# eth-cscs/COSTA

Measured on AMD Instinct MI355X. Metric: GB/s device-resident tile pack+transpose+unpack (fp64), % HBM peak, higher is better.
Workload: dtype f64; 1 GPU; pxtran fp64 16384x16384, 256x256 blocks, op T, alpha=1 beta=0, 1x1 grid (BASELINE configs[1]); op=T, parallelism=1 rank(s), one per GPU, RCCL send/recv exchange, m=16384, n=16384, block=256, grid=1x1

## Files before the change

costa_amd/__init__.py:

```python
from __future__ import annotations

import ctypes as C
import os
import struct
from dataclasses import dataclass
from typing import Iterable, Sequence

import numpy as np

__all__ = [
    "CostaError", "lib", "FLOAT", "DOUBLE", "CFLOAT", "CDOUBLE", "INT32", "HALF", "BFLOAT16",
    "FP8_E4M3", "FP8_E5M2", "FP4_E2M1", "dtype_code", "element_code",
    "np_dtype", "Layout", "block_cyclic_layout", "custom_layout", "Comm", "transform",
    "transform_batch", "transform_async", "transform_batch_async", "synchronize", "transformer", "copy_and_transform", "execute_tiles", "execute_tiles_mixed",
    "convert_subtile", "TileOp", "TriOp", "TRI_OP_DTYPE", "transform_tri", "transform_tri_async",
    "execute_tiles_tri", "plan_export_tri", "tri_cut", "tri_subtile", "tri_phase_ms",
    "plan_export", "set_profiling", "get_stats", "release_caches", "TILE_OP_DTYPE",
    "ScaledOp", "SCALED_OP_DTYPE", "SCALED_F_ROWS", "transform_scaled", "execute_tiles_scaled",
    "plan_export_scaled", "scaled_subtile", "scaled_items",
    "transform_amax", "layout_amax", "execute_tiles_amax", "amax_items",
    "MxScales", "MX_ROWS", "MX_COLS", "MX_FLOOR", "MX_CEIL", "mx_scales", "transform_mx",
    "execute_tiles_mx", "mx_items", "mx_check_ops", "mx_check_scales",
]

# ... 85 lines not shown


class ScaledOp(C.Structure):
    _fields_ = [("op", TileOp), ("row0", C.c_int32), ("col0", C.c_int32)]


MX_ROWS, MX_COLS = 0, 1
MX_FLOOR, MX_CEIL = 0, 1


class MxScales(C.Structure):
    _fields_ = [("data", C.c_void_p), ("axis", C.c_int), ("block_stride", C.c_int64),
                ("line_stride", C.c_int64)]

    def __init__(self, data=0, axis=MX_ROWS, block_stride=0, line_stride=0):
        super().__init__(data, axis, block_stride, line_stride)


class PlanInfo(C.Structure):
    _fields_ = [("n_local", C.c_int64), ("n_pack", C.c_int64), ("n_unpack", C.c_int64),
                ("send_elems", C.c_int64), ("recv_elems", C.c_int64),
                ("local_elems", C.c_int64), ("n_ranks", C.c_int32), ("n_slots", C.c_int32)]


class TriPlanInfo(C.Structure):
    _fields_ = [("base", PlanInfo), ("n_local_tri", C.c_int64), ("n_unpack_tri", C.c_int64)]


class ScaledPlanInfo(C.Structure):
    _fields_ = [("base", PlanInfo), ("n_local_scaled", C.c_int64), ("n_unpack_scaled", C.c_int64)]


class Stats(C.Structure):
    _fields_ = [("pack_ms", C.c_double), ("local_ms", C.c_double), ("unpack_ms", C.c_double),
                ("exchange_ms", C.c_double), ("h2d_ms", C.c_double), ("d2h_ms", C.c_double),
                ("pack_launches", C.c_int64), ("local_launches", C.c_int64),
                ("unpack_launches", C.c_int64), ("pack_bytes", C.c_int64),
                ("local_bytes", C.c_int64), ("unpack_bytes", C.c_int64),
                ("transforms", C.c_int64), ("plan_hits", C.c_int64),
                ("plan_misses", C.c_int64), ("host_groups", C.c_int64),
                ("device_plans", C.c_int64), ("plan_ms", C.c_double), ("host_direct", C.c_int64),
                ("host_direct_groups", C.c_int64), ("tile_items", C.c_int64), ("skew_items", C.c_int64),
                ("cblock_items", C.c_int64), ("tiny_items", C.c_int64), ("device_lists", C.c_int64),
                ("fused_pieces", C.c_int64)]

    def as_dict(self) -> dict:
        out = {}
        for cls in reversed(type(self).__mro__):
            for k, _ in cls.__dict__.get("_fields_", ()):
                out[k] = getattr(self, k)
        return out


class FullStats(Stats):
    _fields_ = [("convert_items", C.c_int64), ("tri_items", C.c_int64)]


LIB_PATH = os.environ.get("COSTA_LIB") or os.path.join(os.path.dirname(os.path.abspath(__file__)),
                                                       "lib", "libcosta_amd.so")
_lib = None


def lib():
    global _lib
    if _lib is not None:
        return _lib
    if not os.environ.get("COSTA_NO_TORCH"):
        try:
            import torch
        except Exception:
            pass
    if not os.path.exists(LIB_PATH):
        raise CostaError(-1, f"native library missing: {LIB_PATH} (run __graft_entry__.build())")
    L = C.CDLL(LIB_PATH, mode=C.RTLD_GLOBAL)
    vp, i, c, i64 = C.c_void_p, C.c_int, C.c_char, C.c_int64
    sig = {
        "costa_hip_last_error": (C.c_char_p, []),
        "costa_hip_version": (i, []),
        "costa_hip_block_cyclic_layout": (i, [i, i, i, i, i, i, i, i, i, i, i, c, i, i, vp, i, c, i,
                                              C.POINTER(vp)]),
        "costa_hip_custom_layout": (i, [i, i, i, C.POINTER(i), C.POINTER(i), C.POINTER(i), i,
                                        C.POINTER(_Block), c, C.POINTER(vp)]),
        "costa_hip_layout_destroy": (None, [vp]),
        "costa_hip_layout_reorder_ranks": (i, [vp, C.POINTER(i), i]),
        "costa_hip_layout_num_blocks": (i, [vp]),
        "costa_hip_layout_shape": (i, [vp, C.POINTER(i), C.POINTER(i)]),
        "costa_hip_layout_block": (i, [vp, i, C.POINTER(i), C.POINTER(i), C.POINTER(i),
                                       C.POINTER(i), C.POINTER(vp), C.POINTER(i)]),
        "costa_hip_comm_self": (i, [i, C.POINTER(vp)]),
        "costa_hip_comm_unique_id": (i, [C.c_char_p]),
        "costa_hip_comm_create": (i, [C.c_char_p, i, i, i, C.POINTER(vp)]),
        "costa_hip_comm_emulated": (i, [i, i, i, C.POINTER(vp)]),
        "costa_hip_comm_emulate": (i, [vp, i, i, vp]),
        "costa_hip_exchange_rounds": (i, []),
        "costa_hip_round_range": (i, [i64, i, i, i, C.POINTER(i64), C.POINTER(i64)]),
        "costa_hip_comm_rank": (i, [vp]),
        "costa_hip_comm_size": (i, [vp]),
        "costa_hip_comm_destroy": (None, [vp]),
        "costa_hip_transform": (i, [vp, vp, c, vp, vp, vp]),
        "costa_hip_transform_batch": (i, [i, C.POINTER(vp), C.POINTER(vp), C.c_char_p, vp, vp,
                                          vp]),
        "costa_hip_transform_async": (i, [vp, vp, c, vp, vp, vp, vp]),
        "costa_hip_transform_batch_async": (i, [i, C.POINTER(vp), C.POINTER(vp), C.c_char_p, vp,
                                                vp, vp, vp]),
        "costa_hip_synchronize": (i, [vp]),
        "costa_hip_device_count": (i, [C.POINTER(i)]),
        "costa_hip_rccl_version": (i, [C.POINTER(i)]),
        "costa_hip_copy_and_transform": (i, [i, i, i, vp, i, i, vp, i, i, i, i, vp, vp]),
        "costa_hip_execute_tiles": (i, [i, C.POINTER(TileOp), i64, vp, vp, vp, i, i]),
        "costa_hip_execute_tiles_mixed": (i, [i, i, C.POINTER(TileOp), i64, vp, vp, vp, i, i]),
        "costa_hip_convert_subtile": (i, [i, i, C.POINTER(i), C.POINTER(i)]),
        "costa_hip_transform_tri": (i, [vp, vp, c, c, i, vp, vp, vp]),
        "costa_hip_transform_tri_async": (i, [vp, vp, c, c, i, vp, vp, vp, vp]),
        "costa_hip_execute_tiles_tri": (i, [i, C.POINTER(TriOp), i64, vp, vp, vp, i, i]),
        "costa_hip_tri_cut": (i, []),
        "costa_hip_tri_phase_ms": (i, [C.POINTER(C.c_double), i]),
        "costa_hip_tri_subtile": (i, [i, C.POINTER(i), C.POINTER(i)]),
        "costa_hip_plan_export_tri": (i, [vp, vp, c, c, i, vp, vp, i, i, C.POINTER(TriPlanInfo), vp, vp,
                                          vp, vp, vp, vp, vp, vp, vp, vp]),
        "costa_hip_transform_scaled": (i, [vp, vp, c, vp, vp, vp, vp, vp]),
        "costa_hip_transform_scaled_async": (i, [vp, vp, c, vp, vp, vp, vp, vp, vp]),
        "costa_hip_execute_tiles_scaled": (i, [i, i, C.POINTER(ScaledOp), i64, vp, vp, vp, i, vp, vp, i]),
        "costa_hip_scaled_subtile": (i, [i, i, C.POINTER(i), C.POINTER(i)]),
        "costa_hip_scaled_items": (i, [C.POINTER(i64), i]),
        "costa_hip_transform_amax": (i, [vp, vp, c, vp, vp, vp, vp, vp, vp, vp]),
        "costa_hip_transform_amax_async": (i, [vp, vp, c, vp, vp, vp, vp, vp, vp, vp, vp]),
        "costa_hip_layout_amax": (i, [vp, vp, vp, vp]),
        "costa_hip_layout_amax_async": (i, [vp, vp, vp, vp, vp]),
        "costa_hip_execute_tiles_amax": (i, [i, i, C.POINTER(ScaledOp), i64, vp, vp, vp, i, vp, vp, vp, vp,
                                             i]),
        "costa_hip_amax_items": (i, [C.POINTER(i64), i]),
        "costa_hip_transform_mx": (i, [vp, vp, c, vp, vp, C.POINTER(MxScales), C.POINTER(MxScales), i, vp]),
        "costa_hip_transform_mx_async": (i, [vp, vp, c, vp, vp, C.POINTER(MxScales), C.POINTER(MxScales), i,
                                             vp, vp]),
        "costa_hip_execute_tiles_mx": (i, [i, i, C.POINTER(ScaledOp), i64, vp, vp, vp, i, C.POINTER(MxScales),
                                           C.POINTER(MxScales), i, i64, i64, i, i]),
        "costa_hip_mx_items": (i, [C.POINTER(i64), i]),
        "costa_hip_mx_check_ops": (i, [C.POINTER(ScaledOp), i64, i, i64, i64]),
        "costa_hip_mx_check_scales": (i, [C.POINTER(MxScales), i64, i64]),
        "costa_hip_plan_export_scaled": (i, [vp, vp, c, vp, vp, i, i, C.POINTER(ScaledPlanInfo), vp, vp,
                                             vp, vp, vp, vp, vp, vp]),
        "costa_hip_plan_export": (i, [i, C.POINTER(vp), C.POINTER(vp), C.c_char_p, vp, vp, i, i,
                                      C.POINTER(PlanInfo), vp, vp, vp, vp, vp, vp, vp, vp]),
        "costa_hip_set_profiling": (i, [i]),
        "costa_hip_get_stats": (i, [C.POINTER(FullStats), i]),
        "costa_hip_release_caches": (i, []),
        "costa_hip_set_host_staging": (i, [i]),
        "costa_hip_set_planner": (i, [i]),
        "costa_hip_plan_export_device": (i, [i, i, C.POINTER(vp), C.POINTER(vp), C.c_char_p, vp, vp,
                                             i, i, C.POINTER(PlanInfo), vp, vp, vp, vp, vp, vp, vp,
                                             vp]),
        "costa_hip_set_list_builder": (i, [i]),
        "costa_hip_work_export": (i, [i, vp, i64, i, i, vp, i64, vp, i64, C.POINTER(i64)]),
    }
    for name, (res, args) in sig.items():
        try:
            f = getattr(L, name)
        except AttributeError:
            if os.environ.get("COSTA_LIB"):
                continue
            raise
        f.restype = res
        f.argtypes = args
    _lib = L
    return L


def _check(rc: int):
    if rc != 0:
        raise CostaError(rc, lib().costa_hip_last_error().decode(errors="replace"))


def _ptr(p) -> int:
    if p is None:
        return 0
    if isinstance(p, int):
        return p
    if isinstance(p, np.ndarray):
        return p.ctypes.data
    if hasattr(p, "data_ptr"):
        return p.data_ptr()
    raise TypeError(f"cannot take the address of {type(p)}")


def _scalar_bytes(code: int, x) -> bytes:
    if code in _FP32_SCALARS:
        code = FLOAT
    if code == DOUBLE:
        return struct.pack("<d", float(x))
    if code == CDOUBLE:
        z = complex(x)
        return struct.pack("<dd", z.real, z.imag)
    return np.asarray(x, dtype=_NP[code]).reshape(1).tobytes()


def _chr(x: str) -> C.c_char:
    return C.c_char(x.encode()[:1])


@dataclass
class BlockInfo:
    row_start: int
    row_end: int
    col_start: int
    col_end: int
    data: int
    ld: int


class Layout:

    def __init__(self, handle: int, dtype: int, keep: Iterable = ()):
        self._h = C.c_void_p(handle)
        self.dtype = dtype
        self._keep = list(keep)

    @property
    def handle(self) -> C.c_void_p:
        return self._h

    def num_blocks(self) -> int:
        return lib().costa_hip_layout_num_blocks(self._h)

    def block(self, i: int) -> BlockInfo:
        v = [C.c_int() for _ in range(4)]
        d, ld = C.c_void_p(), C.c_int()
        _check(lib().costa_hip_layout_block(self._h, i, *[C.byref(x) for x in v], C.byref(d),
                                            C.byref(ld)))
        return BlockInfo(v[0].value, v[1].value, v[2].value, v[3].value, d.value or 0, ld.value)

    def shape(self) -> tuple:
        m, n = C.c_int(), C.c_int()
        _check(lib().costa_hip_layout_shape(self._h, C.byref(m), C.byref(n)))
        return m.value, n.value

    def reorder_ranks(self, reordering: Sequence[int]):
        p = np.ascontiguousarray(reordering, dtype=np.int32)
        _check(lib().costa_hip_layout_reorder_ranks(self._h, p.ctypes.data_as(C.POINTER(C.c_int)),
                                                    int(p.size)))

    def close(self):
        if self._h and self._h.value:
            lib().costa_hip_layout_destroy(self._h)
            self._h = C.c_void_p(0)

    def __del__(self):
        try:
            self.close()
        except Exception:
            pass


def block_cyclic_layout(m, n, block_m, block_n, i, j, sub_m, sub_n, p_m, p_n, order, rsrc, csrc,
                        ptr, lld, ordering, rank, dtype=DOUBLE) -> Layout:
    code = element_code(dtype)
    h = C.c_void_p()
    _check(lib().costa_hip_block_cyclic_layout(code, m, n, block_m, block_n, i, j, sub_m, sub_n,
                                               p_m, p_n, _chr(order), rsrc, csrc,
                                               C.c_void_p(_ptr(ptr)), lld, _chr(ordering), rank,
                                               C.byref(h)))
    return Layout(h.value, code, [ptr])


def custom_layout(rowblocks, colblocks, rowsplit, colsplit, owners, localblocks, ordering,
                  dtype=DOUBLE) -> Layout:
    code = element_code(dtype)
    rs = np.ascontiguousarray(rowsplit, dtype=np.int32)
    cs = np.ascontiguousarray(colsplit, dtype=np.int32)
    ow = np.ascontiguousarray(owners, dtype=np.int32).reshape(-1)
    lb = list(localblocks)
    arr = np.zeros(max(1, len(lb)), _BLOCK_DTYPE)
    if lb:
        arr["data"][:len(lb)] = [_ptr(b[0]) for b in lb]
        rest = np.asarray([b[1:4] for b in lb], dtype=np.int64).reshape(len(lb), 3)
        arr["ld"][:len(lb)] = rest[:, 0]
        arr["row"][:len(lb)] = rest[:, 1]
        arr["col"][:len(lb)] = rest[:, 2]
    h = C.c_void_p()
    ip = C.POINTER(C.c_int)
    _check(lib().costa_hip_custom_layout(code, rowblocks, colblocks, rs.ctypes.data_as(ip),
                                         cs.ctypes.data_as(ip), ow.ctypes.data_as(ip), len(lb),
                                         arr.ctypes.data_as(C.POINTER(_Block)), _chr(ordering),
                                         C.byref(h)))
    return Layout(h.value, code, [b[0] for b in lb])


EMULATE_PACK, EMULATE_UNPACK, EMULATE_LOCAL = 1, 2, 3
EMULATE_PARTS = {"pack": EMULATE_PACK, "unpack": EMULATE_UNPACK, "local": EMULATE_LOCAL}


def exchange_rounds() -> int:
    return lib().costa_hip_exchange_rounds()


def round_range(count: int, elem_bytes: int, rounds: int, round: int) -> tuple:
    lo, hi = C.c_int64(), C.c_int64()
    _check(lib().costa_hip_round_range(count, elem_bytes, rounds, round, C.byref(lo), C.byref(hi)))
    return lo.value, hi.value


class Comm:

    def __init__(self, handle: int):
        self._h = C.c_void_p(handle)

    @staticmethod
# ... 434 lines not shown
        rows, cols = shape
        along, lines = (rows, cols) if ax == MX_ROWS else (cols, rows)
        want = ((along + 31) // 32, lines)
        if tuple(tensor.shape) != want:
            raise ValueError(f"mx_scales: shape {tuple(tensor.shape)}, the matrix needs {want} "
                             "([blocks, lines])")
    bs, ls = tensor.stride()
    if (tensor.shape[0] > 1 and bs <= 0) or (tensor.shape[1] > 1 and ls <= 0):
        raise ValueError("mx_scales: the strides must be positive")
    d = MxScales(tensor.data_ptr(), ax, max(bs, 1), max(ls, 1))
    d._keep = tensor
    return d


def _mx_arg(d, what, shape=None):
    if d is None:
        return None
    if not isinstance(d, MxScales):
        raise ValueError(f"{what}: an MxScales descriptor (costa.mx_scales(tensor, axis)), not {type(d)}")
    t = getattr(d, "_keep", None)
    if t is not None and shape is not None:
        rows, cols = shape
        along, lines = (rows, cols) if d.axis == MX_ROWS else (cols, rows)
        want = ((along + 31) // 32, lines)
        if tuple(t.shape) != want:
            raise ValueError(f"{what}: shape {tuple(t.shape)}, the {rows} x {cols} matrix needs {want} "
                             "([blocks, lines])")
    return C.byref(d)


def transform_mx(A: Layout, Cl: Layout, comm: Comm, trans: str = "N", alpha=1.0, beta=0.0,
                 a_scales=None, c_scales=None, rounding="floor", stream=None):
    if not isinstance(A, Layout) or not isinstance(Cl, Layout):
        raise CostaError(1, "costa: batches of MX layout pairs are not supported")
    code = _scalar_code(A.dtype, Cl.dtype)
    ab, bb = _scalar_bytes(code, alpha), _scalar_bytes(code, beta)
    args = (A.handle, Cl.handle, _chr(trans), ab, bb, _mx_arg(a_scales, "a_scales", A.shape()),
            _mx_arg(c_scales, "c_scales", Cl.shape()), _mx_rounding(rounding), comm.handle)
    if stream is None:
        _check(lib().costa_hip_transform_mx(*args))
    else:
        s = getattr(stream, "cuda_stream", stream) or 0
        _check(lib().costa_hip_transform_mx_async(*args, C.c_void_p(s)))


def execute_tiles_mx(src_dtype, dst_dtype, ops: np.ndarray, scalars: np.ndarray, m: int, n: int,
                     src_base=0, dst_base=0, a_scales=None, c_scales=None, rounding="floor",
                     a_transposed: bool = False, device: int = 0):
    sc_, dc_ = element_code(src_dtype), element_code(dst_dtype)
    ops = np.ascontiguousarray(ops, dtype=SCALED_OP_DTYPE)
    sc = np.ascontiguousarray(scalars, dtype=np.float32).reshape(-1)
    assert sc.size % 2 == 0
    _check(lib().costa_hip_execute_tiles_mx(sc_, dc_, ops.ctypes.data_as(C.POINTER(ScaledOp)), ops.size,
                                            C.c_void_p(_ptr(src_base)), C.c_void_p(_ptr(dst_base)),
                                            sc.ctypes.data, sc.size // 2, _mx_arg(a_scales, "a_scales"),
                                            _mx_arg(c_scales, "c_scales"), _mx_rounding(rounding), m, n,
                                            int(a_transposed), device))


def mx_items(reset: bool = False) -> int:
    v = C.c_int64(0)
    _check(lib().costa_hip_mx_items(C.byref(v), int(reset)))
    return v.value


def mx_check_ops(ops: np.ndarray, axis, m: int, n: int):
    ops = np.ascontiguousarray(ops, dtype=SCALED_OP_DTYPE)
    _check(lib().costa_hip_mx_check_ops(ops.ctypes.data_as(C.POINTER(ScaledOp)), ops.size, _mx_axis(axis),
                                        m, n))


def mx_check_scales(d: MxScales, rows: int, cols: int):
    _check(lib().costa_hip_mx_check_scales(C.byref(d), rows, cols))


@dataclass
class ScaledPlan(Plan):
    local_scaled: np.ndarray = None
    unpack_scaled: np.ndarray = None


def plan_export_scaled(A: Layout, Cl: Layout, rank: int, nranks: int, trans: str = "N", alpha=1,
                       beta=0) -> ScaledPlan:
    if not isinstance(A, Layout) or not isinstance(Cl, Layout):
        raise CostaError(1, "costa: batches of scaled layout pairs are not supported")
    code = _scalar_code(A.dtype, Cl.dtype)
    ab, bb = _scalar_bytes(code, alpha), _scalar_bytes(code, beta)
    info = ScaledPlanInfo()
    L = lib()
    args = (A.handle, Cl.handle, _chr(trans), ab, bb, rank, nranks, C.byref(info))
    _check(L.costa_hip_plan_export_scaled(*args, *([None] * 8)))
    b = info.base
    po = np.zeros(b.n_pack, TILE_OP_DTYPE)
    ls = np.zeros(info.n_local_scaled, SCALED_OP_DTYPE)
    us = np.zeros(info.n_unpack_scaled, SCALED_OP_DTYPE)
    cnt = [np.zeros(nranks, np.int64) for _ in range(4)]
    sc = np.zeros(2 * b.n_slots, _NP[code])
    _check(L.costa_hip_plan_export_scaled(*args, po.ctypes.data, ls.ctypes.data, us.ctypes.data,
                                          *[x.ctypes.data for x in cnt], sc.ctypes.data))
    return ScaledPlan(np.zeros(b.n_local, TILE_OP_DTYPE), po, np.zeros(b.n_unpack, TILE_OP_DTYPE), *cnt,
                      sc, b.send_elems, b.recv_elems, b.local_elems, ls, us)


def set_profiling(on: bool = True):
    _check(lib().costa_hip_set_profiling(int(on)))


def get_stats(reset: bool = False) -> dict:
    s = FullStats()
    _check(lib().costa_hip_get_stats(C.byref(s), int(reset)))
    return s.as_dict()


def release_caches():
    _check(lib().costa_hip_release_caches())


def set_planner(mode: int):
    _check(lib().costa_hip_set_planner(int(mode)))


def set_list_builder(mode: int):
    _check(lib().costa_hip_set_list_builder(int(mode)))


@dataclass
class WorkLists:
    ordered: np.ndarray
    work: np.ndarray
    meta: dict
    on_gpu: bool


_WORK_META = ("n_large", "n_medium", "n_skew", "n_cblock", "cblock_lds", "cb_map", "tiny_first",
              "n_tiny", "n_ordered", "n_work", "on_gpu", "flags")


def work_export(dtype, ops: np.ndarray, kind: str = "local", device=None) -> WorkLists:
    code = element_code(dtype)
    ops = np.ascontiguousarray(ops, dtype=TILE_OP_DTYPE)
    k = {"local": 0, "pack": 1, "unpack": 2}[kind]
    dev = -1 if device is None else int(device)
    meta = (C.c_int64 * 12)()
    L = lib()
    _check(L.costa_hip_work_export(code, ops.ctypes.data, ops.size, k, dev, None, 0, None, 0, meta))
    o = np.zeros(meta[8], TILE_OP_DTYPE)
    w = np.zeros(meta[9], np.uint64)
    _check(L.costa_hip_work_export(code, ops.ctypes.data, ops.size, k, dev, o.ctypes.data, o.size,
                                   w.ctypes.data, w.size, meta))
    m = dict(zip(_WORK_META, list(meta)))
    return WorkLists(o, w, m, bool(m["on_gpu"]))


def set_host_staging(mode: int):
    _check(lib().costa_hip_set_host_staging(int(mode)))


def rccl_version() -> int:
    v = C.c_int(0)
    _check(lib().costa_hip_rccl_version(C.byref(v)))
    return v.value
```

costa_amd/csrc/capi.cpp:

```cpp
#include "engine.hpp"

#include <hip/hip_runtime.h>

#include <costa/transform.hpp>

#include <algorithm>
#include <cctype>
#include <complex>
#include <cstring>
#include <new>

struct costa_layout_s {
    costa::engine::elayout e;
    std::vector<int> base_owners;
};
struct costa_comm_s {
    costa::engine::comm* c = nullptr;
};

namespace {
thread_local std::string g_last_error;

template <typename F>
int guarded(F&& f) {
// ... 695 lines not shown
            throw costa::engine::error(COSTA_ERR_ARG, "bad rank/size");
        check_handles(1, &A, &C);
        auto jobs = make_scaled_job(A, C, trans, alpha, beta, nullptr, nullptr);
        if (costa::engine::dtype_is_fp4(A->e.dtype) || costa::engine::dtype_is_fp4(C->e.dtype)) jobs[0].mx = true;
        auto p = costa::engine::make_plan(jobs, rank, nranks);
        info->base.n_local = int64_t(p->local_ops.size());
        info->base.n_pack = int64_t(p->pack_ops.size());
        info->base.n_unpack = int64_t(p->unpack_ops.size());
        info->base.send_elems = p->send_elems;
        info->base.recv_elems = p->recv_elems;
        info->base.local_elems = p->local_elems;
        info->base.n_ranks = nranks;
        info->base.n_slots = int32_t(p->slots.size());
        info->n_local_scaled = int64_t(p->local_scaled.size());
        info->n_unpack_scaled = int64_t(p->unpack_scaled.size());
        auto cp = [](const auto& v, auto* dst) {
            if (dst && !v.empty()) std::memcpy(dst, v.data(), v.size() * sizeof(v[0]));
        };
        cp(p->pack_ops, pack_ops);
        cp(p->local_scaled, local_scaled);
        cp(p->unpack_scaled, unpack_scaled);
        cp(p->send_counts, send_counts);
        cp(p->send_displs, send_displs);
        cp(p->recv_counts, recv_counts);
        cp(p->recv_displs, recv_displs);
        if (scalars) {
            const size_t E = dtype_size(p->scalar_dtype());
            auto* out = static_cast<unsigned char*>(scalars);
            std::memcpy(out, p->slots[0].alpha.data(), E);
            std::memcpy(out + E, p->slots[0].beta.data(), E);
        }
    });
}

int costa_hip_synchronize(costa_comm_t comm) {
    return gpu_guarded([&] {
        if (!comm) throw costa::engine::error(COSTA_ERR_ARG, "null communicator");
        costa::engine::synchronize(comm->c);
    });
}

int costa_hip_copy_and_transform(costa_dtype_t dtype, int n_rows, int n_cols, const void* src,
                                 int src_stride, int src_col_major, void* dst, int dst_stride,
                                 int dst_col_major, int transpose, int conjugate,
                                 const void* alpha, const void* beta) {
    return gpu_guarded([&] {
        if (!alpha || !beta) throw costa::engine::error(COSTA_ERR_ARG, "null scalar");
        costa::engine::copy_and_transform(dtype, n_rows, n_cols, src, src_stride, src_col_major != 0,
                                          dst, dst_stride, dst_col_major != 0, transpose != 0,
                                          conjugate != 0, alpha, beta);
    });
}

int costa_hip_execute_tiles(costa_dtype_t dtype, const costa_tile_op_t* ops, int64_t n,
                            const void* src_base, void* dst_base, const void* scalars,
                            int n_slots, int device) {
    return gpu_guarded([&] {
        if (n < 0 || (n > 0 && (!ops || !scalars)))
            throw costa::engine::error(COSTA_ERR_ARG, "null argument");
        costa::engine::execute_tiles(dtype, ops, n, src_base, dst_base, scalars, n_slots, device);
    });
}

int costa_hip_execute_tiles_mixed(costa_dtype_t src_dtype, costa_dtype_t dst_dtype,
                                  const costa_tile_op_t* ops, int64_t n, const void* src_base,
                                  void* dst_base, const void* scalars, int n_slots, int device) {
    return gpu_guarded([&] {
        if (n < 0 || (n > 0 && (!ops || !scalars)))
            throw costa::engine::error(COSTA_ERR_ARG, "null argument");
        costa::engine::execute_tiles_mixed(src_dtype, dst_dtype, ops, n, src_base, dst_base, scalars,
                                           n_slots, device);
    });
}

int costa_hip_convert_subtile(costa_dtype_t src_dtype, costa_dtype_t dst_dtype, int* bf, int* bs) {
    return guarded([&] {
        if (!bf || !bs) throw costa::engine::error(COSTA_ERR_ARG, "null argument");
        costa::engine::convert_subtile(src_dtype, dst_dtype, bf, bs);
    });
}

int costa_hip_plan_export(int n, const costa_layout_t* A, const costa_layout_t* C,
                          const char* trans, const void* alpha, const void* beta, int rank,
                          int nranks, costa_plan_info_t* info, costa_tile_op_t* local_ops,
                          costa_tile_op_t* pack_ops, costa_tile_op_t* unpack_ops,
                          int64_t* send_counts, int64_t* send_displs, int64_t* recv_counts,
                          int64_t* recv_displs, void* scalars) {
    return export_plan(
        [&](const std::vector<job>& jobs) { return costa::engine::make_plan(jobs, rank, nranks); },
        n, A, C, trans, alpha, beta, rank, nranks, info, local_ops, pack_ops, unpack_ops,
        send_counts, send_displs, recv_counts, recv_displs, scalars);
}

int costa_hip_plan_export_device(int device, int n, const costa_layout_t* A, const costa_layout_t* C,
                                 const char* trans, const void* alpha, const void* beta, int rank,
                                 int nranks, costa_plan_info_t* info, costa_tile_op_t* local_ops,
                                 costa_tile_op_t* pack_ops, costa_tile_op_t* unpack_ops,
                                 int64_t* send_counts, int64_t* send_displs, int64_t* recv_counts,
                                 int64_t* recv_displs, void* scalars) {
    device_restore keep;
    return export_plan(
        [&](const std::vector<job>& jobs) {
            auto p = costa::engine::make_plan_device(jobs, rank, nranks, 0, device, nullptr);
            if (!p)
                throw costa::engine::error(COSTA_ERR_ARG,
                                           "costa: the device planner does not apply to these "
                                           "layouts (local blocks are not exactly the rank's grid "
                                           "cells)");
            return p;
        },
        n, A, C, trans, alpha, beta, rank, nranks, info, local_ops, pack_ops, unpack_ops,
        send_counts, send_displs, recv_counts, recv_displs, scalars);
}

int costa_hip_set_planner(int mode) {
    return guarded([&] {
        if (mode < 0 || mode > 2) throw costa::engine::error(COSTA_ERR_ARG, "mode must be 0, 1 or 2");
        costa::engine::set_planner_mode(mode);
    });
}

int costa_hip_set_list_builder(int mode) {
    return guarded([&] {
        if (mode < 0 || mode > 2) throw costa::engine::error(COSTA_ERR_ARG, "mode must be 0, 1 or 2");
        costa::engine::set_list_builder_mode(mode);
    });
}

int costa_hip_work_export(int dtype, const costa_tile_op_t* ops, int64_t n_ops, int kind, int device,
                          costa_tile_op_t* ordered, int64_t cap_ordered, uint64_t* work,
                          int64_t cap_work, int64_t* meta) {
    auto body = [&] {
        if (!meta || (n_ops > 0 && !ops) || n_ops < 0) throw costa::engine::error(COSTA_ERR_ARG, "null argument");
        if (dtype < COSTA_FLOAT || dtype > COSTA_INT32) throw costa::engine::error(COSTA_ERR_ARG, "bad dtype");
        if (kind < 0 || kind > 2) throw costa::engine::error(COSTA_ERR_ARG, "kind must be 0, 1 or 2");
        std::vector<costa_tile_op_t> in(ops, ops + n_ops), o;
        std::vector<uint64_t> w;
        costa::engine::work_split ws;
        const bool on_gpu = costa::engine::work_export(
            costa_dtype_t(dtype), in, costa::engine::list_kind(kind), device, o, w, ws);
        const int64_t m[12] = {ws.n_large, ws.n_medium, ws.n_skew, ws.n_cblock, ws.cblock_lds, ws.cb_map,
                               ws.tiny_first, ws.n_tiny, int64_t(o.size()), int64_t(w.size()), on_gpu,
                               int64_t(ws.tr_shape) | int64_t(ws.sq) << 1 | int64_t(ws.full) << 2 |
                                   int64_t(ws.med_full) << 3 | int64_t(ws.med_sq) << 4 |
                                   int64_t(ws.skew_wide) << 5};
        std::memcpy(meta, m, sizeof(m));
        if (ordered && cap_ordered >= int64_t(o.size()) && !o.empty())
            std::memcpy(ordered, o.data(), o.size() * sizeof(o[0]));
        if (work && cap_work >= int64_t(w.size()) && !w.empty()) std::memcpy(work, w.data(), w.size() * sizeof(w[0]));
    };
    return device >= 0 ? gpu_guarded(body) : guarded(body);
}

int costa_hip_set_profiling(int on) {
    costa::engine::set_profiling(on != 0);
    return COSTA_OK;
}

int costa_hip_get_stats(costa_stats_t* out, int reset) {
    return guarded([&] {
        if (!out) throw costa::engine::error(COSTA_ERR_ARG, "null argument");
        costa::engine::resolve_pending();
        *out = costa::engine::stats();
        if (reset) costa::engine::stats() = costa_stats_t{};
    });
}

int costa_hip_set_host_staging(int mode) {
    return guarded([&] {
        if (mode != 0 && mode != 1) throw costa::engine::error(COSTA_ERR_ARG, "mode must be 0 or 1");
        costa::engine::set_host_staging_mode(mode);
    });
}

int costa_hip_release_caches(void) {
    return gpu_guarded([&] { costa::engine::release_caches(); });
}

}

namespace costa {
namespace {
void raise(int rc) {
    if (rc != COSTA_OK) throw hip_error(rc, g_last_error);
}
template <typename T>
engine::scal scal_of(T a, T b) {
    engine::scal s;
    std::memcpy(s.alpha.data(), &a, sizeof(T));
    std::memcpy(s.beta.data(), &b, sizeof(T));
    return s;
}
template <typename T>
void run(std::vector<layout_ref<T>>& from, std::vector<layout_ref<T>>& to, const char* trans,
         const T* alpha, const T* beta, costa_comm_t comm) {
    raise(gpu_guarded([&] {
        if (from.size() != to.size())
            throw engine::error(COSTA_ERR_ARG, "costa::transform: from/to sizes differ");
        if (!comm) throw engine::error(COSTA_ERR_ARG, "costa::transform: null communicator");
        std::vector<engine::elayout> es;
        es.reserve(2 * from.size());
        std::vector<engine::job> jobs(from.size());
        for (size_t i = 0; i < from.size(); ++i) {
            es.push_back(engine::erase(from[i].get()));
            jobs[i].A = &es.back();
            es.push_back(engine::erase(to[i].get()));
            jobs[i].C = &es.back();
            jobs[i].trans = trans ? trans[i] : 'N';
            jobs[i].s = alpha ? scal_of(alpha[i], beta[i]) : scal_of(T{1}, T{0});
        }
        engine::transform(jobs, comm->c);
    }));
}
}

template <typename T>
void transform(grid_layout<T>& A, grid_layout<T>& C, costa_comm_t comm) {
    std::vector<layout_ref<T>> f{A}, t{C};
    run<T>(f, t, nullptr, nullptr, nullptr, comm);
}

template <typename T>
void transform(grid_layout<T>& A, grid_layout<T>& C, char trans, T alpha, T beta,
               costa_comm_t comm) {
    std::vector<layout_ref<T>> f{A}, t{C};
    run<T>(f, t, &trans, &alpha, &beta, comm);
}

template <typename T>
void transform(std::vector<layout_ref<T>>& from, std::vector<layout_ref<T>>& to,
               costa_comm_t comm) {
    run<T>(from, to, nullptr, nullptr, nullptr, comm);
}

template <typename T>
void transform(std::vector<layout_ref<T>>& from, std::vector<layout_ref<T>>& to, const char* trans,
               const T* alpha, const T* beta, costa_comm_t comm) {
    run<T>(from, to, trans, alpha, beta, comm);
}

template <typename T>
void transform_triangular(grid_layout<T>& A, grid_layout<T>& C, char trans, char uplo, int k, T alpha,
                          T beta, costa_comm_t comm) {
    raise(gpu_guarded([&] {
        if (!comm) throw engine::error(COSTA_ERR_ARG, "costa::transform_triangular: null communicator");
        const char ul = char(std::toupper(static_cast<unsigned char>(uplo)));
        if (ul != 'U' && ul != 'L')
            throw engine::error(COSTA_ERR_ARG, "costa::transform_triangular: uplo must be 'U' or 'L'");
        engine::elayout a = engine::erase(A), c = engine::erase(C);
        engine::job jb;
        jb.A = &a;
        jb.C = &c;
        jb.trans = trans;
        jb.s = scal_of(alpha, beta);
        jb.uplo = ul;
        jb.k = k;
        engine::transform({jb}, comm->c);
    }));
}
#define COSTA_INSTANTIATE_TRI(T)                                                                  \
    template void transform_triangular<T>(grid_layout<T>&, grid_layout<T>&, char, char, int, T, T, \
                                          costa_comm_t);
COSTA_INSTANTIATE_TRI(float)
COSTA_INSTANTIATE_TRI(double)
COSTA_INSTANTIATE_TRI(std::complex<float>)
COSTA_INSTANTIATE_TRI(std::complex<double>)
COSTA_INSTANTIATE_TRI(int)

template <typename Ta, typename Tc>
void run_mixed(grid_layout<Ta>& A, grid_layout<Tc>& C, char trans, Tc alpha, Tc beta,
               costa_comm_t comm) {
    raise(gpu_guarded([&] {
        if (!comm) throw engine::error(COSTA_ERR_ARG, "costa::transform: null communicator");
        engine::elayout a = engine::erase(A), c = engine::erase(C);
        engine::job jb;
        jb.A = &a;
        jb.C = &c;
        jb.trans = trans;
        jb.s = scal_of(alpha, beta);
        engine::transform({jb}, comm->c);
    }));
}

template <typename Ta, typename Tc>
typename std::enable_if<!std::is_same<Ta, Tc>::value>::type
transform(grid_layout<Ta>& A, grid_layout<Tc>& C, costa_comm_t comm) {
    run_mixed<Ta, Tc>(A, C, 'N', Tc{1}, Tc{0}, comm);
}

template <typename Ta, typename Tc>
typename std::enable_if<!std::is_same<Ta, Tc>::value>::type
transform(grid_layout<Ta>& A, grid_layout<Tc>& C, char trans, Tc alpha, Tc beta, costa_comm_t comm) {
    run_mixed<Ta, Tc>(A, C, trans, alpha, beta, comm);
}

#define COSTA_INSTANTIATE_MIXED(Ta, Tc)                                                         \
    template void transform<Ta, Tc>(grid_layout<Ta>&, grid_layout<Tc>&, costa_comm_t);          \
    template void transform<Ta, Tc>(grid_layout<Ta>&, grid_layout<Tc>&, char, Tc, Tc, costa_comm_t);

COSTA_INSTANTIATE_MIXED(double, float)
COSTA_INSTANTIATE_MIXED(float, double)
COSTA_INSTANTIATE_MIXED(std::complex<double>, std::complex<float>)
COSTA_INSTANTIATE_MIXED(std::complex<float>, std::complex<double>)

#define COSTA_INSTANTIATE_TRANSFORM(T)                                                          \
    template void transform<T>(grid_layout<T>&, grid_layout<T>&, costa_comm_t);                 \
// ... 14 lines not shown
```

costa_amd/csrc/device_lists.hip:

```cpp
#include <hip/hip_runtime.h>
#include <rocprim/device/device_radix_sort.hpp>
#include <rocprim/device/device_scan.hpp>
#include <rocprim/device/device_scan_by_key.hpp>

#include <algorithm>
#include <chrono>
#include <cstdio>
#include <cstdlib>

#include "engine.hpp"

namespace costa {
namespace engine {

#define DL_CHECK(x)                                                                    \
    do {                                                                               \
        hipError_t e_ = (x);                                                           \
        if (e_ != hipSuccess)                                                          \
            throw error(COSTA_ERR_HIP, std::string(#x " failed: ") + hipGetErrorString(e_)); \
    } while (0)

namespace {

using u64 = unsigned long long;
// ... 530 lines not shown
    DL_CHECK(hipMemcpyAsync(d_ops, ops_h.data(), ops_h.size() * sizeof(costa_tile_op_t), hipMemcpyHostToDevice, s));
    DL_CHECK(hipMemcpyAsync(d_wave, wave_h.data(), N * 4, hipMemcpyHostToDevice, s));
    DL_CHECK(hipMemcpyAsync(d_t, &th, sizeof(th), hipMemcpyHostToDevice, s));
    DL_CHECK(hipMemsetAsync(odd, 0, N * 4, s));
    DL_CHECK(hipMemsetAsync(bad, 0, N * 4, s));
    DL_CHECK(hipMemsetAsync(taken, 0, N, s));
    hipLaunchKernelGGL(dl_candidates, dim3(dl_grid(nw)), dim3(kThreads), 0, s, d_ops, d_wave, nw, E, budget, flag,
                       lo, hi, ldd, d_t);
    DL_CHECK(hipGetLastError());
    scan_u32(flag, pos, N);
    hipLaunchKernelGGL(dl_compact, dim3(dl_grid(nw)), dim3(kThreads), 0, s, flag, pos, nw, cand, d_t);
    DL_CHECK(hipGetLastError());
    DL_CHECK(hipMemcpyAsync(&th, d_t, sizeof(th), hipMemcpyDeviceToHost, s));
    sync();
    lap[0] = now() - t0;
    const int64_t nc = int64_t(th.ncand);
    if (nc < 2) return 0;
    const uint64_t lo_min = th.lo_min;
    const int sb = bits_of((th.lo_max - lo_min) / uint64_t(E)), lb = bits_of(uint64_t(budget));
    const int hb = bits_of((th.hi_max - lo_min) / uint64_t(E));
    if (sb + lb > 64 || hb + lb > 64) return -1;
    const size_t NC = size_t(nc);

    hipLaunchKernelGGL(dl_keys, dim3(dl_grid(nc)), dim3(kThreads), 0, s, cand, nc, lo, ldd, lo_min, E, sb, key, va);
    DL_CHECK(hipGetLastError());
    sort_u64(key, NC, sb + lb, sval, ka, kb, va, vb);
    hipLaunchKernelGGL(dl_gather, dim3(dl_grid(nc)), dim3(kThreads), 0, s, sval, cand, d_wave, nc, lo, hi, ldd, s_i,
                       s_op, s_lo, s_hi, s_ldd);
    hipLaunchKernelGGL(dl_rhi, dim3(dl_grid(nc)), dim3(kThreads), 0, s, s_ldd, s_hi, nc, lo_min, E, hb, rhi);
    DL_CHECK(hipGetLastError());
    max_u64(rhi, pmax, NC);
    hipLaunchKernelGGL(dl_starts, dim3(dl_grid(nc)), dim3(kThreads), 0, s, s_lo, s_ldd, pmax, nc, lo_min, E, hb,
                       start);
    DL_CHECK(hipGetLastError());
    scan_u32(start, cnum, NC);
    hipLaunchKernelGGL(dl_inclusive, dim3(dl_grid(nc)), dim3(kThreads), 0, s, start, nc, cnum);
    hipLaunchKernelGGL(dl_bounds, dim3(dl_grid(nc)), dim3(kThreads), 0, s, start, cnum, nc, comp_a, comp_b, d_t);
    hipLaunchKernelGGL(dl_check, dim3(dl_grid(nc)), dim3(kThreads), 0, s, d_ops, s_op, s_lo, s_ldd, comp_a, comp_b, nc,
                       E, vec_bits, comp_K, comp_fl, comp_ok, d_t);
    DL_CHECK(hipGetLastError());
    DL_CHECK(hipMemcpyAsync(&th, d_t, sizeof(th), hipMemcpyDeviceToHost, s));
    sync();
    lap[1] = now() - t0;
    const uint64_t ncomp = th.ncomp;
    if (th.ck_max == 0) return 0;
    const int ck = bits_of(th.ck_max), cb = bits_of(ncomp);
    if (ck + cb > 64) return -1;

    hipLaunchKernelGGL(dl_corners, dim3(dl_grid(nc)), dim3(kThreads), 0, s, d_ops, s_op, s_lo, s_ldd, cnum, comp_a,
                       comp_ok, comp_K, nc, E, ck, ncomp, ckeys);
    DL_CHECK(hipGetLastError());
    sort_u64(ckeys, 4 * NC, ck + cb, perm, ka, kb, va, vb);
    hipLaunchKernelGGL(dl_gather_u64, dim3(dl_grid(4 * nc)), dim3(kThreads), 0, s, ckeys, perm, 4 * nc, sckeys);
    hipLaunchKernelGGL(dl_parity, dim3(dl_grid(4 * nc)), dim3(kThreads), 0, s, sckeys, 4 * nc, ck, ncomp, s_ldd,
                       comp_a, comp_K, odd, bad);
    hipLaunchKernelGGL(dl_count, dim3(dl_grid(nc)), dim3(kThreads), 0, s, comp_ok, odd, bad, s_ldd, comp_a, comp_K,
                       budget, nc, comp_ng, comp_KB, d_t);
    DL_CHECK(hipGetLastError());
    scan_i64(comp_ng, comp_gat, NC);
    hipLaunchKernelGGL(dl_total, dim3(1), dim3(64), 0, s, comp_ng, comp_gat, d_t);
    DL_CHECK(hipGetLastError());
    DL_CHECK(hipMemcpyAsync(&th, d_t, sizeof(th), hipMemcpyDeviceToHost, s));
    sync();
    lap[2] = now() - t0;
    const int64_t ng = int64_t(th.ng);
    if (ng == 0) return 0;
    if (ng > int64_t(UINT32_MAX)) return -1;
    const size_t G = size_t(ng);

    dl_mem mg;
    const size_t o_gc = mg.take(G * 8), o_gc2 = mg.take(G * 8), o_gd = mg.take(G * 8), o_gb = mg.take(G * 4);
    const size_t o_gn = mg.take(G * 4), o_gh = mg.take(G * 4), o_gk = mg.take(G * 8);
    const size_t o_io = mg.take(G * 4), o_o1 = mg.take(G * 4), o_by = mg.take(G * 4), o_sh = mg.take(G * 4);
    const size_t o_bd = mg.take(G * 4), o_bk = mg.take(G * 4), o_sbk = mg.take(G * 4), o_ord = mg.take(G * 4);
    const size_t o_sz = mg.take(G * 8), o_at = mg.take(G * 8);
    const size_t o_gka = mg.take(G * 4), o_gkb = mg.take(G * 4), o_gva = mg.take(G * 4), o_gvb = mg.take(G * 4);
    mg.alloc();
    uint64_t *g_comp0 = mg.at<uint64_t>(o_gc), *g_comp = mg.at<uint64_t>(o_gc2), *g_dst = mg.at<uint64_t>(o_gd);
    uint32_t *g_band = mg.at<uint32_t>(o_gb), *g_nops = mg.at<uint32_t>(o_gn), *g_hint = mg.at<uint32_t>(o_gh);
    uint64_t* gkey = mg.at<uint64_t>(o_gk);
    uint32_t *iota = mg.at<uint32_t>(o_io), *order1 = mg.at<uint32_t>(o_o1), *by = mg.at<uint32_t>(o_by);
    uint32_t *shint = mg.at<uint32_t>(o_sh), *slice = mg.at<uint32_t>(o_bd), *bkey = mg.at<uint32_t>(o_bk);
    uint32_t *sbkey = mg.at<uint32_t>(o_sbk), *order = mg.at<uint32_t>(o_ord);
    uint64_t *gsize = mg.at<uint64_t>(o_sz), *gat = mg.at<uint64_t>(o_at);
    uint32_t *gka = mg.at<uint32_t>(o_gka), *gkb = mg.at<uint32_t>(o_gkb), *gva = mg.at<uint32_t>(o_gva);
    uint32_t* gvb = mg.at<uint32_t>(o_gvb);

    DL_CHECK(hipMemsetAsync(g_comp0, 0, G * 8, s));
    hipLaunchKernelGGL(dl_seed, dim3(dl_grid(nc)), dim3(kThreads), 0, s, comp_ng, comp_gat, nc, g_comp0, d_t);
    DL_CHECK(hipGetLastError());
    max_u64(g_comp0, g_comp, G);
    hipLaunchKernelGGL(dl_table, dim3(dl_grid(ng)), dim3(kThreads), 0, s, d_ops, s_op, s_lo, s_ldd, comp_a, comp_b,
                       comp_K, comp_KB, comp_fl, comp_gat, g_comp, ng, E, g_dst, g_band, g_nops, g_hint, d_t);
    hipLaunchKernelGGL(dl_taken, dim3(dl_grid(nc)), dim3(kThreads), 0, s, cnum, comp_ng, s_i, nc, taken);
    hipLaunchKernelGGL(dl_dst_keys, dim3(dl_grid(ng)), dim3(kThreads), 0, s, g_dst, ng, lo_min, E, gkey, iota);
    DL_CHECK(hipGetLastError());
    sort_u64(gkey, G, hb, order1, gka, gkb, gva, gvb);
    DL_CHECK(hipMemcpyAsync(&th, d_t, sizeof(th), hipMemcpyDeviceToHost, s));
    sync();
    lap[3] = now() - t0;
    const bool any_tr = th.any_tr != 0, hints = th.hints_bad == 0;
    lds = int64_t(th.lds);
    map = any_tr ? cb_xcd_chunks : cb_round_robin;
    const bool bands = bands_env == 1 || (bands_env == -1 && !any_tr);
    const uint32_t* final_order = order1;
    if (bands && ng >= 16 && hints) {
        hipLaunchKernelGGL(dl_iota, dim3(dl_grid(ng)), dim3(kThreads), 0, s, ng, iota);
        DL_CHECK(hipGetLastError());
        sort_u32(g_hint, shint, iota, by, G, 32);
        hipLaunchKernelGGL(dl_slices, dim3(dl_grid(ng)), dim3(kThreads), 0, s, by, ng, slice);
        hipLaunchKernelGGL(dl_gather_u32, dim3(dl_grid(ng)), dim3(kThreads), 0, s, slice, order1, ng, bkey);
        DL_CHECK(hipGetLastError());
        sort_u32(bkey, sbkey, order1, order, G, 3);
        final_order = order;
        map = cb_xcd_bands;
    }

    hipLaunchKernelGGL(dl_sizes, dim3(dl_grid(ng)), dim3(kThreads), 0, s, final_order, g_nops, ng, gsize);
    DL_CHECK(hipGetLastError());
    scan_i64(gsize, gat, G);
    hipLaunchKernelGGL(dl_out_total, dim3(1), dim3(64), 0, s, gat, gsize, ng, d_t);
    DL_CHECK(hipGetLastError());
    DL_CHECK(hipMemcpyAsync(&th, d_t, sizeof(th), hipMemcpyDeviceToHost, s));
    sync();
    lap[4] = now() - t0;
    const size_t n_out = size_t(th.n_out);
    void* out = nullptr;
    const size_t out_ops_bytes = (n_out * sizeof(costa_tile_op_t) + 255) & ~size_t(255);
    DL_CHECK(hipMalloc(&out, out_ops_bytes + G * 8));
    sec.mem = std::shared_ptr<void>(out, [](void* p) { (void)hipFree(p); });
    sec.d_ordered = static_cast<costa_tile_op_t*>(out);
    sec.d_work = reinterpret_cast<uint64_t*>(static_cast<char*>(out) + out_ops_bytes);
    hipLaunchKernelGGL(dl_emit, dim3(dl_grid(ng)), dim3(kThreads), 0, s, d_ops, s_op, s_lo, s_ldd, comp_a, comp_b,
                       comp_K, comp_KB, comp_fl, g_comp, g_band, g_nops, g_dst, final_order, gat, ng, E,
                       uint64_t(base_at), sec.d_ordered, sec.d_work);
    DL_CHECK(hipGetLastError());
    DL_CHECK(hipMemcpyAsync(taken_h.data(), taken, N, hipMemcpyDeviceToHost, s));
    sync();
    sec.at_ordered = base_at;
    sec.n_ordered = n_out;
    sec.n_work = G;
    if (trace) {
        lap[5] = now() - t0;
        std::fprintf(stderr,
                     "[costa device groups] %lld candidates, %llu components (%llu / %llu checked, %llu stray, %llu four), %lld groups: upload + candidates "
                     "%.2f ms, order + components + check %.2f, corners + counts %.2f, group table + order "
                     "%.2f, slices + sizes %.2f, emit %.2f\n",
                     (long long)nc, (unsigned long long)ncomp, th.n_ok, th.n_valid, th.n_bad, th.n_odd4, (long long)ng, lap[0], lap[1] - lap[0],
                     lap[2] - lap[1], lap[3] - lap[2], lap[4] - lap[3], lap[5] - lap[4]);
    }
    return ng;
}

}
}
```

costa_amd/csrc/engine.cpp:

```cpp
#include <exception>
#include <thread>
#include "engine.hpp"
#include "strip_work.hpp"

#include <hip/hip_runtime.h>
#include <rccl/rccl.h>

#include <algorithm>
#include <numeric>
#include <chrono>
#include <cmath>
#include <cstdio>
#include <cstdlib>
#include <cstring>
#include <deque>
#include <list>
#include <map>
#include <mutex>
#include <unordered_map>

namespace costa {
namespace engine {

#define HIP_CHECK(x)                                                                   \
// ... 1239 lines not shown
                key[x] = {((op.dst + uint64_t((fp * op.ldd + s0) * E)) << 6) | uint64_t((f0 - fp) / bf), wx};
            }
            std::sort(key.begin(), key.end());
            const size_t n = key.size(), blk = size_t(8 * F);
            for (size_t b = 0; b < n; b += blk) {
                const size_t m = std::min(blk, n - b);
                for (size_t x = 0; x < m; ++x) {
                    const size_t run = x / size_t(F), in = x % size_t(F);
                    const size_t to = m == blk ? in * 8 + run : x;
                    work[w0 + b + to] = key[b + x].second;
                }
            }
        }
        n_work[c] = int64_t(work.size() - w0);
    }
    lap(0);
    int64_t cblock_lds = 0;
    int cb_map = cb_round_robin;
    const int64_t n_cblock = cblock_groups(dtype, wave_ops, kind, ordered, work, cblock_lds, cb_map, ops, dev);
    const size_t n_dev = dev ? dev->n_ordered : 0;
    lap(1);
    const size_t nw = wave_ops.size();
    uint32_t top = 0;
    bool tr = false;
    for (const auto* o : wave_ops) {
        top = std::max(top, o->order);
        tr = tr || (o->flags & COSTA_TILE_TRANSPOSE);
    }
    const int mode = kn.sort == 5   ? (pack_list ? 1 : 2)
                     : kn.sort == 4 ? (tr || top == 0 ? 2 : 3)
                     : kn.sort == 3 && top == 0 ? 2 : kn.sort;
    std::vector<uint32_t> perm(nw);
    if (mode == 3 && size_t(top) <= 4 * nw + 1024) {
        std::vector<uint32_t> at(size_t(top) + 2, 0);
        for (const auto* o : wave_ops) ++at[size_t(o->order) + 1];
        for (size_t k = 1; k < at.size(); ++k) at[k] += at[k - 1];
        for (size_t i = 0; i < nw; ++i) perm[at[wave_ops[i]->order]++] = uint32_t(i);
    } else if (mode == 2 && nw > 0) {
        uint64_t lo = ~uint64_t(0), hi = 0;
        for (const auto* o : wave_ops) {
            lo = std::min(lo, o->dst);
            hi = std::max(hi, o->dst);
        }
        std::vector<uint64_t> key(nw), key2(nw);
        std::vector<uint32_t> idx2(nw);
        for (size_t i = 0; i < nw; ++i) {
            key[i] = (wave_ops[i]->dst - lo) / uint64_t(E);
            perm[i] = uint32_t(i);
        }
        const uint64_t span = (hi - lo) / uint64_t(E);
        constexpr int B = 14;
        std::vector<uint32_t> at((1 << B) + 1);
        for (int shift = 0; shift == 0 || (shift < 64 && (span >> shift) != 0); shift += B) {
            std::fill(at.begin(), at.end(), 0u);
            for (size_t i = 0; i < nw; ++i) ++at[((key[i] >> shift) & ((1 << B) - 1)) + 1];
            for (int d = 1; d <= (1 << B); ++d) at[d] += at[d - 1];
            for (size_t i = 0; i < nw; ++i) {
                const uint32_t p = at[(key[i] >> shift) & ((1 << B) - 1)]++;
                key2[p] = key[i];
                idx2[p] = perm[i];
            }
            key.swap(key2);
            perm.swap(idx2);
        }
    } else if (mode >= 1 && mode <= 3) {
        std::vector<std::pair<uint64_t, uint32_t>> key(nw);
        for (size_t i = 0; i < nw; ++i) {
            const costa_tile_op_t& o = *wave_ops[i];
            key[i] = {mode == 1 ? o.src : mode == 2 ? o.dst : o.order, uint32_t(i)};
        }
        std::sort(key.begin(), key.end());
        for (size_t i = 0; i < nw; ++i) perm[i] = key[i].second;
    } else {
        for (size_t i = 0; i < nw; ++i) perm[i] = uint32_t(i);
    }
    if (kn.xcd_bands && mode == 2 && top > 0 && nw > 1) xcd_bands(wave_ops, E, kn.xcd_bands, local, perm);
    lap(2);
    std::vector<wave_grid> grid(nw);
    std::vector<size_t> at_piece(nw + 1, 0);
    host_parallel(nw, [&](size_t b, size_t e) {
        for (size_t i = b; i < e; ++i) grid[i] = wave_pieces(*wave_ops[perm[i]], E, local);
    });
    for (size_t i = 0; i < nw; ++i)
        at_piece[i + 1] = at_piece[i] + size_t(grid[i].nfc * grid[i].nsc);
    work_split w;
    w.tr_shape = tr_shape;
    w.sq = sq;
    w.full = tr_shape && !sq && !shaped[0].empty();
    for (const uint32_t li : shaped[0]) {
        const costa_tile_op_t& op = ops[li];
        w.full = w.full && (op.flags & vec_both) == vec_both && op.nf % sh.bf == 0 && op.ns % sh.bs == 0;
    }
    w.med_sq = med_sq && !shaped[1].empty();
    w.med_full = !shaped[1].empty() && n_work[1] > 0 && !w.med_sq;
    for (const uint32_t li : shaped[1])
        w.med_full = w.med_full && ops[li].nf % sh.bf_m == 0 && ops[li].ns % sh.bs_m == 0;
    w.n_large = n_work[0];
    w.n_medium = n_work[1];
    w.n_skew = n_work[2];
    w.skew_wide = skew_wide && n_work[2] > 0;
    w.n_cblock = n_cblock;
    w.cblock_lds = cblock_lds;
    w.cb_map = cb_map;

    w.tiny_first = int64_t(ordered.size() + n_dev);
    w.n_tiny = int64_t(at_piece[nw]);
    const size_t base = ordered.size();
    ordered.resize(base + at_piece[nw]);
    host_parallel(nw, [&](size_t b, size_t e) {
        for (size_t i = b; i < e; ++i)
            emit_pieces(*wave_ops[perm[i]], E, grid[i], local, &ordered[base + at_piece[i]]);
    });
    if (trace) {
        lap(3);
        std::fprintf(stderr,
                     "[costa build_work] %zu ops (%s list): classify + shaped %.2f ms (merge %.2f, flags + "
                     "granules %.2f, classify %.2f, work items %.2f), groups %.2f (%lld), "
                     "wavefront order %.2f, pieces %.2f (%lld)\n",
                     ops_in.size(), pack_list ? "pack" : local ? "local" : "unpack", bw_t[0], sub_t[0],
                     sub_t[1] - sub_t[0], sub_t[2] - sub_t[1], bw_t[0] - sub_t[2], bw_t[1] - bw_t[0],
                     (long long)n_cblock, bw_t[2] - bw_t[1], bw_t[3] - bw_t[2], (long long)w.n_tiny);
    }
    return w;
}

launch_args make_launch(const work_split& w, const void* d_ordered, const void* d_work,
                        const char* src_base, char* dst_base, const void* d_scalars, bool transpose,
                        bool axpby) {
    launch_args a;
    a.ops = static_cast<const costa_tile_op_t*>(d_ordered);
    a.work = static_cast<const uint64_t*>(d_work);
    a.n_large = w.n_large;
    a.n_medium = w.n_medium;
    a.n_skew = w.n_skew;
    a.n_cblock = w.n_cblock;
    a.cblock_lds = w.cblock_lds;
    a.cb_map = w.cb_map;
    a.tiny_first = w.tiny_first;
    a.n_tiny = w.n_tiny;
    a.src_base = src_base;
    a.dst_base = dst_base;
    a.scalars = d_scalars;
    a.any_transpose = transpose;
    a.any_axpby = axpby;
    a.tr_shape = w.tr_shape;
    a.sq = w.sq;
    a.full = w.full;
    a.med_full = w.med_full;
    a.med_sq = w.med_sq;
    a.skew_wide = w.skew_wide;
    return a;
}

namespace {

struct hrange {
    uintptr_t lo, hi;
    size_t dev_off;
};

size_t block_extent_bytes(const eblock& b, char ordering, size_t E) {
    const int64_t nr = b.rows.length(), nc = b.cols.length();
    if (nr == 0 || nc == 0) return 0;
    const int64_t fast = ordering == 'R' ? nc : nr, slow = ordering == 'R' ? nr : nc;
    return size_t((slow - 1) * int64_t(b.ld) + fast) * E;
}

bool is_device_ptr(const void* p) {
    hipPointerAttribute_t a;
    hipError_t e = hipPointerGetAttributes(&a, p);
    if (e != hipSuccess) {
        (void)hipGetLastError();
        return false;
    }
    return a.type == hipMemoryTypeDevice;
}

bool layout_on_device(const elayout& L) {
    if (L.blocks.empty()) return true;
    bool first = is_device_ptr(L.blocks.front().data);
    uintptr_t lo = 0, hi = 0;
    for (const auto& b : L.blocks) {
        uintptr_t p = reinterpret_cast<uintptr_t>(b.data);
        if (first && p >= lo && p < hi) continue;
        bool d = is_device_ptr(b.data);
        if (d != first)
            throw error(COSTA_ERR_ARG, "costa: a layout mixes host and device blocks");
        if (d) {
            hipDeviceptr_t base = nullptr;
            size_t sz = 0;
            if (hipMemGetAddressRange(&base, &sz, const_cast<char*>(b.data)) == hipSuccess) {
                lo = reinterpret_cast<uintptr_t>(base);
                hi = lo + sz;
            } else {
                (void)hipGetLastError();
            }
        }
    }
    return first;
}

}

namespace {
int g_host_mode = -1;
}
int host_staging_mode() {
    if (g_host_mode < 0) {
        const char* s = std::getenv("COSTA_HOST_STAGING");
        g_host_mode = s ? (std::atoi(s) != 0) : 1;
    }
    return g_host_mode;
}
void set_host_staging_mode(int mode) {
    std::lock_guard<std::recursive_mutex> lk(g_mutex);
    g_host_mode = mode != 0;
}

namespace {

struct hasher {
    uint64_t h = 0x9E3779B97F4A7C15ull;
    uint64_t h2 = 0x2545F4914F6CDD1Dull;
    void mix(uint64_t v) {
        v ^= v >> 33;
        v *= 0xff51afd7ed558ccdull;
        v ^= v >> 33;
        h = (h ^ v) * 0xc4ceb9fe1a85ec53ull + 0x165667b19e3779f9ull;
        h ^= h >> 29;
        h2 = (h2 + v) * 0x9fb21c651e98df25ull;
        h2 ^= h2 >> 31;
    }
    void mix_vec(const std::vector<int>& v) {
        mix(v.size());
        for (int x : v) mix(uint64_t(uint32_t(x)));
    }
    void mix_layout(const elayout& L) {
        mix(uint64_t(L.dtype));
        mix(uint64_t(uint8_t(L.ordering)));
        mix(uint64_t(L.n_ranks));
        mix_vec(L.rows_split);
        mix_vec(L.cols_split);
        mix_vec(L.owners);
        mix(L.blocks.size());
        for (const auto& b : L.blocks) {
            mix(uint64_t(uint32_t(b.rows.start)) | (uint64_t(uint32_t(b.rows.end)) << 32));
            mix(uint64_t(uint32_t(b.cols.start)) | (uint64_t(uint32_t(b.cols.end)) << 32));
            mix(reinterpret_cast<uintptr_t>(b.data));
            mix(uint64_t(uint32_t(b.ld)));
        }
    }
};

}

uint64_t layout_hash(const elayout& L) {
    hasher h;
    h.mix_layout(L);
    return h.h | 1;
}

void layout_hashes(const elayout& L, uint64_t& h1, uint64_t& h2) {
    hasher h;
    h.mix_layout(L);
    h1 = h.h | 1;
    h2 = h.h2;
}

void set_layout_hash(elayout& L) { layout_hashes(L, L.hash, L.hash2); }

namespace {

struct cached_plan {
    std::unique_ptr<plan> p;
    int device = 0;
    bool staged = false;
    std::vector<hrange> h2d_ranges, d2h_ranges;
    dbuf stage;
    dbuf d_local, w_local, d_scal;
    work_split l_local;
    bool tr_local = true, ax_local = true;
    strip_list c_local;
    dbuf d_local_tri, w_local_tri;
    strip_list t_local;
    dbuf d_local_sc, w_local_sc;
    strip_list s_local;
    int mx_rule[2] = {0, 0};
    struct xround {
        dbuf d_pack, w_pack, d_unpack, w_unpack;
        work_split l_pack, l_unpack;
        strip_list c_pack, c_unpack;
        dbuf d_unpack_tri, w_unpack_tri;
        strip_list t_unpack;
        dbuf d_unpack_sc, w_unpack_sc;
        strip_list s_unpack;
        bool tr_unpack = false, ax_unpack = false;
    };
    std::vector<std::unique_ptr<xround>> rounds;
    std::vector<unsigned char> scal_host;
    std::shared_ptr<host_pipeline> pipe;
};

constexpr size_t kMaxPlans = 16;
struct keyed_plan {
    uint64_t h = 0;
    std::vector<uint64_t> key;
    std::unique_ptr<cached_plan> plan;
};
std::list<keyed_plan> g_plans;

void key_layout(std::vector<uint64_t>& k, const elayout& L) {
    uint64_t h1 = L.hash, h2 = L.hash2;
    if (!h1) layout_hashes(L, h1, h2);
    k.push_back(h1);
    k.push_back(h2);
    k.push_back(uint64_t(L.dtype) | uint64_t(uint8_t(L.ordering)) << 8 |
                uint64_t(uint32_t(L.n_ranks)) << 32);
    k.push_back(uint64_t(uint32_t(L.nbr())) | uint64_t(uint32_t(L.nbc())) << 32);
    k.push_back(L.blocks.size());
    if (!L.blocks.empty())
        for (const eblock* b : {&L.blocks.front(), &L.blocks.back()}) {
            k.push_back(reinterpret_cast<uintptr_t>(b->data));
            k.push_back(uint64_t(uint32_t(b->ld)) | uint64_t(uint32_t(b->rows.start)) << 32);
        }
}

elayout remap(const elayout& L, const std::vector<hrange>& ranges, char* dev) {
    elayout out = L;
    for (auto& b : out.blocks) {
        uintptr_t p = reinterpret_cast<uintptr_t>(b.data);
        auto it = std::upper_bound(ranges.begin(), ranges.end(), p,
                                   [](uintptr_t v, const hrange& r) { return v < r.lo; });
        if (it == ranges.begin()) throw error(COSTA_ERR_INTERNAL, "costa: staging map miss");
        --it;
        b.data = dev + it->dev_off + (p - it->lo);
    }
    return out;
}

std::vector<hrange> collect_ranges(const std::vector<const elayout*>& Ls) {
    std::vector<hrange> r;
    for (const elayout* L : Ls) {
        const size_t E = dtype_size(L->dtype);
        for (const auto& b : L->blocks) {
            size_t ext = block_extent_bytes(b, L->ordering, E);
            if (!ext) continue;
            uintptr_t lo = reinterpret_cast<uintptr_t>(b.data);
            r.push_back({lo, lo + ext, 0});
        }
    }
    std::sort(r.begin(), r.end(), [](const hrange& x, const hrange& y) { return x.lo < y.lo; });
    std::vector<hrange> m;
    for (const auto& x : r) {
        if (!m.empty() && x.lo <= m.back().hi)
            m.back().hi = std::max(m.back().hi, x.hi);
        else
            m.push_back(x);
    }
    return m;
}

}

namespace {
int g_planner = -1;
constexpr size_t kDevicePlanBlocks = 4096;
constexpr size_t kColdDevicePlanBlocks = 100000;
bool g_device_planner_warm = false;
}

int planner_mode() {
    if (g_planner < 0) {
        const char* s = std::getenv("COSTA_PLANNER");
        g_planner = s ? std::max(0, std::min(2, std::atoi(s))) : 1;
    }
    return g_planner;
}

void set_planner_mode(int mode) {
    std::lock_guard<std::recursive_mutex> lk(g_mutex);
    g_planner = mode;
}

namespace {
int g_list_builder = -1;
}

int list_builder_mode() {
    if (g_list_builder < 0) {
        const char* s = std::getenv("COSTA_LIST_BUILDER");
        g_list_builder = s ? std::max(0, std::min(2, std::atoi(s))) : 1;
    }
    return g_list_builder;
}

void set_list_builder_mode(int mode) {
    std::lock_guard<std::recursive_mutex> lk(g_mutex);
    g_list_builder = mode;
}

namespace {
template <typename X>
void upload_list(dbuf& d, const std::vector<X>& h, const X* sec, size_t at, size_t n, hipStream_t s) {
    if (!sec || n == 0) return d.upload(h, s);
    const size_t total = h.size() + n;
    d.reserve(total * sizeof(X));
    X* p = static_cast<X*>(d.p);
    if (at) HIP_CHECK(hipMemcpyAsync(p, h.data(), at * sizeof(X), hipMemcpyHostToDevice, s));
    HIP_CHECK(hipMemcpyAsync(p + at, sec, n * sizeof(X), hipMemcpyDeviceToDevice, s));
    if (h.size() > at)
        HIP_CHECK(hipMemcpyAsync(p + at + n, h.data() + at, (h.size() - at) * sizeof(X), hipMemcpyHostToDevice, s));
}
}

bool work_export(costa_dtype_t dtype, const std::vector<costa_tile_op_t>& ops, list_kind kind, int device,
                 std::vector<costa_tile_op_t>& ordered, std::vector<uint64_t>& work, work_split& w) {
    std::lock_guard<std::recursive_mutex> lk(g_mutex);
    if (device < 0) {
        w = build_work(dtype, ops, ordered, work, kind);
        return false;
    }
    device_ctx& dc = ctx(device);
    device_section sec;
    sec.device = device;
    sec.stream = dc.main;
    sec.force = true;
    w = build_work(dtype, ops, ordered, work, kind, &sec);
    if (!sec.n_ordered) return false;
    std::vector<costa_tile_op_t> o(sec.n_ordered);
    std::vector<uint64_t> k(sec.n_work);
    HIP_CHECK(hipMemcpyAsync(o.data(), sec.d_ordered, o.size() * sizeof(o[0]), hipMemcpyDeviceToHost, dc.main));
    HIP_CHECK(hipMemcpyAsync(k.data(), sec.d_work, k.size() * sizeof(k[0]), hipMemcpyDeviceToHost, dc.main));
    HIP_CHECK(hipStreamSynchronize(dc.main));
    ordered.insert(ordered.begin() + std::ptrdiff_t(sec.at_ordered), o.begin(), o.end());
    work.insert(work.begin() + std::ptrdiff_t(sec.at_work), k.begin(), k.end());
    return true;
}

namespace {
std::unique_ptr<plan> plan_jobs(const std::vector<job>& jobs, comm* c, hipStream_t s) {
    const int lb = c->size == 1 && c->nccl ? loopback_exchange() : 0;
    const int mode = planner_mode();
    size_t blocks = 0;
    for (const job& j : jobs) blocks += j.A->blocks.size() + j.C->blocks.size();
    const size_t need = g_device_planner_warm ? kDevicePlanBlocks : kColdDevicePlanBlocks;
    if (!any_fp4(jobs) && (mode == 2 || (mode == 1 && blocks >= need))) {
        if (auto p = make_plan_device(jobs, c->rank, c->size, lb, c->device, s)) {
            g_stats.device_plans++;
            g_device_planner_warm = true;
            return p;
        }
    }
    return make_plan(jobs, c->rank, c->size, lb);
}

costa_dtype_t pack_src(const plan& p) { return dtype_is_fp4(p.src_dtype) ? COSTA_FP8_E4M3 : p.src_dtype; }
costa_dtype_t pack_dst(const plan& p) { return dtype_is_fp4(p.pkg_dtype) ? COSTA_FP8_E4M3 : p.pkg_dtype; }

cached_plan* get_plan(const std::vector<job>& jobs, comm* c, device_ctx& dc) {
    std::vector<uint64_t> key;
    key.reserve(4 + jobs.size() * 30);
    key.push_back(uint64_t(uint32_t(c->rank)) | uint64_t(uint32_t(c->size)) << 32);
    key.push_back(uint64_t(uint32_t(c->device)) | uint64_t(uint32_t(host_staging_mode())) << 32);
    key.push_back(jobs.size());
    for (const auto& j : jobs) {
        key_layout(key, *j.A);
        key_layout(key, *j.C);
        uint64_t w = uint64_t(uint8_t(std::toupper(static_cast<unsigned char>(j.trans))));
        for (bool cm : {true, false})
            w = w << 8 | scale_kind(j.C->dtype, j.s, cm, std::toupper(j.trans) == 'C');
        key.push_back(w);
        key.push_back(uint64_t(uint8_t(std::toupper(static_cast<unsigned char>(j.uplo)))) << 32 |
                      uint64_t(j.scaled) << 40 | uint64_t(uint32_t(j.k)));
    }
    hasher h;
    for (uint64_t w : key) h.mix(w);
    for (auto it = g_plans.begin(); it != g_plans.end(); ++it) {
        if (it->h == h.h && it->key == key) {
            g_plans.splice(g_plans.begin(), g_plans, it);
            g_stats.plan_hits++;
            return g_plans.front().plan.get();
        }
    }
    g_stats.plan_misses++;
    static const bool trace = std::getenv("COSTA_PLAN_TRACE") != nullptr;
    auto now = [] {
        return std::chrono::duration<double, std::milli>(
                   std::chrono::steady_clock::now().time_since_epoch()).count();
    };
    const double t0 = now();
    double t_resid = 0, t_plan = 0, t_work = 0;

    const bool half = any_half(jobs);
    const bool fp8 = any_fp8(jobs);
    const bool fp4 = any_fp4(jobs);
    const bool mixed = any_mixed(jobs) || half || fp8 || fp4;
    const bool masked = any_masked(jobs);
    const bool scaled = any_scaled(jobs);
    if (mixed || masked || scaled) {
        costa_dtype_t a, b;
        check_jobs(jobs, c->size, a, b);
    }
    auto cp = std::make_unique<cached_plan>();
    cp->device = c->device;
    bool all_dev = true;
    std::vector<const elayout*> host_layouts;
    std::vector<bool> on_dev;
    for (const auto& j : jobs)
        for (const elayout* L : {j.A, j.C}) {
            bool d = layout_on_device(*L);
            on_dev.push_back(d);
            all_dev = all_dev && d;
        }
    std::vector<elayout> remapped;
    std::vector<job> pj = jobs;
    std::vector<hrange> staged_ranges;
    std::vector<uint8_t> range_flags;
    if (!all_dev && mixed)
        throw error(COSTA_ERR_ARG,
                    fp4  ? "costa: FP4 transforms (A or C of the packed 4-bit element type) need "
                           "device-resident layouts"
                    : fp8 ? "costa: FP8 transforms (A or C of a 1-byte element type) need "
                           "device-resident layouts"
                    : half ? "costa: half-precision transforms (A or C of a 2-byte element type) need "
                           "device-resident layouts"
                         : "costa: mixed-precision transforms (A and C of different element types) need "
                           "device-resident layouts");
    if (!all_dev && scaled)
        throw error(COSTA_ERR_ARG, "costa: scaled transforms need device-resident layouts");
    if (!all_dev) {
        cp->staged = true;
        std::vector<const elayout*> As, Cs;
        size_t k = 0;
        for (const auto& j : jobs) {
            if (!on_dev[k++]) As.push_back(j.A);
            if (!on_dev[k++]) Cs.push_back(j.C);
        }
        std::vector<const elayout*> all = As;
        all.insert(all.end(), Cs.begin(), Cs.end());
        auto ranges = collect_ranges(all);
        size_t off = 0;
        for (auto& r : ranges) {
            r.dev_off = off;
            off += ((r.hi - r.lo) + 255) & ~size_t(255);
        }
        range_flags.assign(ranges.size(), 0);
        std::vector<int> c_job(ranges.size(), -1);
        auto range_of = [&](uintptr_t p) {
            auto it = std::upper_bound(ranges.begin(), ranges.end(), p,
                                       [](uintptr_t v, const hrange& r) { return v < r.lo; });
            return size_t(it - ranges.begin()) - 1;
        };
        k = 0;
        for (size_t t = 0; t < jobs.size(); ++t) {
            const bool a_host = !on_dev[k++], c_host = !on_dev[k++];
            for (int side = 0; side < 2; ++side) {
                if (!(side == 0 ? a_host : c_host)) continue;
                const elayout* L = side == 0 ? jobs[t].A : jobs[t].C;
                const size_t E = dtype_size(L->dtype);
                for (const auto& b : L->blocks) {
                    if (!block_extent_bytes(b, L->ordering, E)) continue;
                    const size_t i = range_of(reinterpret_cast<uintptr_t>(b.data));
                    if (side == 0) {
                        range_flags[i] |= 1;
                    } else {
                        range_flags[i] |= 2;
                        if (c_job[i] >= 0 && c_job[i] != int(t)) range_flags[i] |= 4;
                        c_job[i] = int(t);
                    }
                }
            }
        }
        bool pipe_ok = host_staging_mode() == 1 && !masked &&
                       std::none_of(on_dev.begin(), on_dev.end(), [](bool d) { return d; });
        for (uint8_t f : range_flags)
            if ((f & 3) == 3 || (f & 4)) pipe_ok = false;
        if (pipe_ok) {
            const double tp = now();
            auto hplan = plan_jobs(jobs, c, dc.main);
            g_stats.plan_ms += now() - tp;
            if (host_pipeline_accepts(hplan->dtype, hplan->pack_ops)) {
                cp->staged = false;
                cp->p = std::move(hplan);
                const int R = c->exchanges() ? exchange_rounds() : 1;
                std::vector<int> pr, ur;
                exchange_round_of_ops(*cp->p, R, pr, ur);
                cp->pipe = make_host_pipeline(cp->p->dtype, cp->p->pack_ops, cp->p->local_ops,
                                              cp->p->unpack_ops, pr, ur, R);
                g_plans.push_front({h.h, std::move(key), std::move(cp)});
                while (g_plans.size() > kMaxPlans) g_plans.pop_back();
                return g_plans.front().plan.get();
            }
        }
        cp->stage.reserve(std::max<size_t>(off, 256));
        staged_ranges = ranges;
        remapped.reserve(jobs.size() * 2);
        k = 0;
        for (auto& j : pj) {
            if (!on_dev[k++]) {
                remapped.push_back(remap(*j.A, ranges, static_cast<char*>(cp->stage.p)));
                j.A = &remapped.back();
            }
            if (!on_dev[k++]) {
                remapped.push_back(remap(*j.C, ranges, static_cast<char*>(cp->stage.p)));
                j.C = &remapped.back();
            }
        }
    }
    t_resid = now() - t0;
    cp->p = plan_jobs(pj, c, dc.main);
    const plan& p = *cp->p;
    t_plan = now() - t0 - t_resid;
    g_stats.plan_ms += t_plan;
    if (cp->staged) {
        const size_t E = dtype_size(p.dtype);
        const uintptr_t base = reinterpret_cast<uintptr_t>(cp->stage.p);
        std::vector<size_t> written(staged_ranges.size(), 0);
        std::vector<bool> reads_c(staged_ranges.size(), false);
        auto account = [&](const std::vector<costa_tile_op_t>& ops) {
            for (const auto& op : ops) {
                if (op.dst < base) continue;
                const size_t off = size_t(op.dst - base);
                auto it = std::upper_bound(staged_ranges.begin(), staged_ranges.end(), off,
                                           [](size_t v, const hrange& r) { return v < r.dev_off; });
                if (it == staged_ranges.begin()) continue;
                const size_t i = size_t(it - staged_ranges.begin()) - 1;
                if (off >= staged_ranges[i].dev_off + (staged_ranges[i].hi - staged_ranges[i].lo))
                    continue;
                written[i] += size_t(op.nf) * size_t(op.ns) * E;
                if (((op.flags & COSTA_SCALE_MASK) >> COSTA_SCALE_SHIFT) == COSTA_SCALE_AXPBY)
                    reads_c[i] = true;
            }
        };
        account(p.local_ops);
        account(p.unpack_ops);
        for (size_t i = 0; i < staged_ranges.size(); ++i) {
            const hrange& r = staged_ranges[i];
            const uint8_t f = range_flags[i];
            const bool overwritten = !masked && f == 2 && !reads_c[i] && written[i] == r.hi - r.lo;
            if ((f & 1) || ((f & 2) && !overwritten)) cp->h2d_ranges.push_back(r);
            if (f & 2) cp->d2h_ranges.push_back(r);
        }
    }
    cp->tr_local = any_transpose(p.local_ops);
    cp->ax_local = any_axpby(p.local_ops);
    std::vector<costa_tile_op_t> ord_l;
    std::vector<uint64_t> w_l;
    auto section = [&] {
        device_section d;
        d.device = c->device;
        d.stream = dc.main;
        return d;
    };
    device_section sec_l = section();
    const bool cv_pack = p.half() || (p.fp4()   ? dtype_is_fp4(p.src_dtype)
                                      : p.fp8() ? dtype_is_fp8(p.src_dtype)
                                                : p.mixed() && p.pkg_dtype != p.src_dtype);
    const bool cv_unpack = !p.fp4() && (p.half() || p.fp8() || (p.mixed() && p.pkg_dtype != p.dtype));
    if (p.fp4()) {
        if (!p.local_ops.empty() || !p.unpack_ops.empty())
            throw error(COSTA_ERR_INTERNAL, "costa: an FP4 plan with ordinary LOCAL / UNPACK ops");
    } else if (p.converting())
        cp->c_local = build_convert_work(p.src_dtype, p.dtype, p.local_ops, 0, 0, ord_l, w_l);
    else
        cp->l_local = build_work(p.dtype, p.local_ops, ord_l, w_l, list_local, &sec_l, masked);
    std::vector<costa_tri_op_t> ord_lt;
    std::vector<uint64_t> w_lt;
    if (!p.local_tri.empty()) cp->t_local = build_tri_work(p.dtype, p.local_tri, 0, 0, ord_lt, w_lt);
    std::vector<costa_scaled_op_t> ord_ls;
    std::vector<uint64_t> w_ls;
    if (!p.local_scaled.empty()) {
        static const bool by_dst = [] {
            const char* e = tuning_env("COSTA_SCALED_ORDER");
            return !e || std::atoi(e) != 0;
        }();
        cp->s_local = build_scaled_work(p.src_dtype, p.dtype, p.local_scaled, 0, 0, ord_ls, w_ls, by_dst);
    }
    const int R = c->exchanges() ? exchange_rounds() : 1;
    std::vector<std::vector<costa_tile_op_t>> pk(static_cast<size_t>(R)), up(static_cast<size_t>(R));
    {
        std::vector<int> pr, ur;
        exchange_round_of_ops(p, R, pr, ur);
        for (size_t i = 0; i < p.pack_ops.size(); ++i) pk[size_t(pr[i])].push_back(p.pack_ops[i]);
        for (size_t i = 0; i < p.unpack_ops.size(); ++i) up[size_t(ur[i])].push_back(p.unpack_ops[i]);
    }
    std::vector<std::vector<costa_tri_op_t>> upt(static_cast<size_t>(R)), ord_ut(static_cast<size_t>(R));
    std::vector<std::vector<uint64_t>> w_ut(static_cast<size_t>(R));
    if (!p.unpack_tri.empty()) {
        std::vector<int> tr;
        exchange_round_of_tri(p, R, tr);
        for (size_t i = 0; i < p.unpack_tri.size(); ++i) upt[size_t(tr[i])].push_back(p.unpack_tri[i]);
    }
    std::vector<std::vector<costa_scaled_op_t>> ups(static_cast<size_t>(R)), ord_us(static_cast<size_t>(R));
    std::vector<std::vector<uint64_t>> w_us(static_cast<size_t>(R));
    if (!p.unpack_scaled.empty()) {
        std::vector<int> sr;
        exchange_round_of_scaled(p, R, sr);
        for (size_t i = 0; i < p.unpack_scaled.size(); ++i) ups[size_t(sr[i])].push_back(p.unpack_scaled[i]);
    }
    std::vector<std::vector<costa_tile_op_t>> ord_p(static_cast<size_t>(R)), ord_u(static_cast<size_t>(R));
    std::vector<std::vector<uint64_t>> w_p(static_cast<size_t>(R)), w_u(static_cast<size_t>(R));
    std::vector<device_section> sec_u(static_cast<size_t>(R), section());
    for (int r = 0; r < R; ++r) {
        auto x = std::make_unique<cached_plan::xround>();
        x->tr_unpack = any_transpose(up[size_t(r)]);
        x->ax_unpack = any_axpby(up[size_t(r)]);
        if (cv_pack)
            x->c_pack = build_convert_work(pack_src(p), pack_dst(p), pk[size_t(r)], 0, 0, ord_p[size_t(r)],
                                           w_p[size_t(r)]);
        else
            x->l_pack = build_work(p.pkg_dtype, pk[size_t(r)], ord_p[size_t(r)], w_p[size_t(r)], list_pack);
        if (cv_unpack)
            x->c_unpack = build_convert_work(p.pkg_dtype, p.dtype, up[size_t(r)], 0, 0, ord_u[size_t(r)],
                                             w_u[size_t(r)]);
        else if (!p.fp4())
            x->l_unpack = build_work(p.dtype, up[size_t(r)], ord_u[size_t(r)], w_u[size_t(r)], list_unpack,
                                     &sec_u[size_t(r)]);
        if (!upt[size_t(r)].empty())
            x->t_unpack = build_tri_work(p.dtype, upt[size_t(r)], 0, 0, ord_ut[size_t(r)], w_ut[size_t(r)]);
        if (!ups[size_t(r)].empty())
            x->s_unpack = build_scaled_work(p.pkg_dtype, p.dtype, ups[size_t(r)], 0, 0, ord_us[size_t(r)],
                                            w_us[size_t(r)], false);
        cp->rounds.push_back(std::move(x));
    }
    t_work = now() - t0 - t_resid - t_plan;
    upload_list(cp->d_local, ord_l, sec_l.d_ordered, sec_l.at_ordered, sec_l.n_ordered, dc.main);
    upload_list(cp->w_local, w_l, sec_l.d_work, sec_l.at_work, sec_l.n_work, dc.main);
    if (cp->t_local.n_items) {
        cp->d_local_tri.upload(ord_lt, dc.main);
        cp->w_local_tri.upload(w_lt, dc.main);
    }
    if (cp->s_local.n_items) {
        cp->d_local_sc.upload(ord_ls, dc.main);
        cp->w_local_sc.upload(w_ls, dc.main);
    }
    for (int r = 0; r < R; ++r) {
        auto& x = *cp->rounds[size_t(r)];
        const device_section& su = sec_u[size_t(r)];
        if (x.s_unpack.n_items) {
            x.d_unpack_sc.upload(ord_us[size_t(r)], dc.main);
            x.w_unpack_sc.upload(w_us[size_t(r)], dc.main);
        }
        x.d_pack.upload(ord_p[size_t(r)], dc.main);
        x.w_pack.upload(w_p[size_t(r)], dc.main);
        upload_list(x.d_unpack, ord_u[size_t(r)], su.d_ordered, su.at_ordered, su.n_ordered, dc.main);
        upload_list(x.w_unpack, w_u[size_t(r)], su.d_work, su.at_work, su.n_work, dc.main);
        if (x.t_unpack.n_items) {
            x.d_unpack_tri.upload(ord_ut[size_t(r)], dc.main);
            x.w_unpack_tri.upload(w_ut[size_t(r)], dc.main);
        }
    }
    HIP_CHECK(hipStreamSynchronize(dc.main));
    if (trace)
        std::fprintf(stderr,
                     "[costa plan] %zu local / %zu pack / %zu unpack ops: residency %.2f ms, "
                     "planning %.2f, work lists %.2f, upload %.2f, total %.2f\n",
                     p.local_ops.size(), p.pack_ops.size(), p.unpack_ops.size(), t_resid, t_plan,
                     t_work, now() - t0 - t_resid - t_plan - t_work, now() - t0);

    g_plans.push_front({h.h, std::move(key), std::move(cp)});
    while (g_plans.size() > kMaxPlans) g_plans.pop_back();
    return g_plans.front().plan.get();
}

void upload_scalars(cached_plan& cp, const std::vector<job>& jobs, hipStream_t s) {
    const size_t E = dtype_size(cp.p->scalar_dtype());
    std::vector<unsigned char> host(jobs.size() * 2 * E);
    for (size_t t = 0; t < jobs.size(); ++t) {
        std::memcpy(&host[(2 * t) * E], jobs[t].s.alpha.data(), E);
        std::memcpy(&host[(2 * t + 1) * E], jobs[t].s.beta.data(), E);
    }
    if (host != cp.scal_host || !cp.d_scal.p) {
        cp.d_scal.reserve(host.size());
        cp.scal_host = host;
        HIP_CHECK(hipMemcpyAsync(cp.d_scal.p, cp.scal_host.data(), host.size(),
                                 hipMemcpyHostToDevice, s));
    }
}

}

void release_caches() {
    std::lock_guard<std::recursive_mutex> lk(g_mutex);
    g_plans.clear();
    release_host_rings();
    ctx_map().clear();
}

namespace {
enum phase { PH_LOCAL, PH_PACK, PH_EXCHANGE, PH_UNPACK, PH_H2D, PH_D2H, PH_TRI_LOCAL, PH_TRI_UNPACK };
double g_tri_ms = 0;
int64_t g_scaled_items = 0;
int64_t g_amax_items = 0;
int64_t g_mx_items = 0;

struct phase_timer {
    device_ctx& dc;
    bool on;
    int ph = 0;
    hipEvent_t a = nullptr;
    hipStream_t s = nullptr;
    phase_timer(device_ctx& d, bool prof) : dc(d), on(prof) {}
    void start(int p, hipStream_t st) {
        if (!on) return;
        ph = p;
        s = st;
        a = dc.take_event();
        HIP_CHECK(hipEventRecord(a, s));
    }
    void stop() {
        if (!on || !a) return;
        hipEvent_t b = dc.take_event();
        HIP_CHECK(hipEventRecord(b, s));
        dc.pending.push_back({ph, a, b});
        a = nullptr;
        if (dc.pending.size() > 1024) dc.resolve(64);
    }
};
}

void device_ctx::resolve(size_t max_n) {
    size_t n = 0;
    while (!pending.empty() && n < max_n) {
        timed t = pending.front();
        pending.pop_front();
        float ms = 0.f;
        HIP_CHECK(hipEventSynchronize(t.b));
        HIP_CHECK(hipEventElapsedTime(&ms, t.a, t.b));
        double* acc[] = {&g_stats.local_ms, &g_stats.pack_ms, &g_stats.exchange_ms,
                         &g_stats.unpack_ms, &g_stats.h2d_ms, &g_stats.d2h_ms};
        if (t.phase == PH_TRI_LOCAL || t.phase == PH_TRI_UNPACK) {
            (t.phase == PH_TRI_LOCAL ? g_stats.local_ms : g_stats.unpack_ms) += ms;
            g_tri_ms += ms;
        } else {
            *acc[t.phase] += ms;
        }
        free_events.push_back(t.a);
        free_events.push_back(t.b);
        ++n;
    }
}

hipEvent_t device_ctx::take_event() {
    if (free_events.empty()) {
        hipEvent_t e;
        HIP_CHECK(hipEventCreate(&e));
        return e;
    }
    hipEvent_t e = free_events.back();
    free_events.pop_back();
    return e;
}

void resolve_pending() {
    std::lock_guard<std::recursive_mutex> lk(g_mutex);
    for (auto& kv : ctx_map()) {
        HIP_CHECK(hipSetDevice(kv.first));
        kv.second->resolve();
    }
}

double tri_phase_ms(bool reset) {
    resolve_pending();
    std::lock_guard<std::recursive_mutex> lk(g_mutex);
    const double v = g_tri_ms;
    if (reset) g_tri_ms = 0;
    return v;
}

void synchronize(comm* c) {
    std::lock_guard<std::recursive_mutex> lk(g_mutex);
    if (!c) throw error(COSTA_ERR_ARG, "costa: null communicator");
    device_ctx& dc = ctx(c->device);
    HIP_CHECK(hipStreamSynchronize(dc.main));
    HIP_CHECK(hipStreamSynchronize(dc.aux));
    HIP_CHECK(hipStreamSynchronize(dc.xch));
    dc.resolve();
}

namespace {
void issue_exchange(comm* c, const plan& p, char* sb, char* rb, hipStream_t s, int round = 0,
                    int rounds = 1) {
    const size_t E = pkg_unit_size(p.pkg_dtype);
    const size_t piece = max_message_bytes();
    NCCL_CHECK(ncclGroupStart());
    for (int q = 0; q < c->size; ++q) {
        int64_t slo, shi, rlo, rhi;
        round_range(p.send_counts[size_t(q)], E, rounds, round, slo, shi);
        round_range(p.recv_counts[size_t(q)], E, rounds, round, rlo, rhi);
        const size_t sbytes = size_t(shi - slo) * E, rbytes = size_t(rhi - rlo) * E;
        char* sp = sb + size_t(p.send_displs[size_t(q)] + slo) * E;
        char* rp = rb + size_t(p.recv_displs[size_t(q)] + rlo) * E;
        for (size_t o = 0; o < sbytes; o += piece)
            NCCL_CHECK(ncclSend(sp + o, std::min(piece, sbytes - o), ncclUint8, q, c->nccl, s));
        for (size_t o = 0; o < rbytes; o += piece)
            NCCL_CHECK(ncclRecv(rp + o, std::min(piece, rbytes - o), ncclUint8, q, c->nccl, s));
    }
    NCCL_CHECK(ncclGroupEnd());
}

struct scaled_args {
    const void *row_scale = nullptr, *col_scale = nullptr;
    void *row_amax = nullptr, *col_amax = nullptr;
    bool amax() const { return row_amax || col_amax; }
    bool mx = false;
    mx_side a_scales, c_scales;
    bool ceil = false;
};

void layout_extent(const elayout& L, int64_t& rows, int64_t& cols) {
    rows = L.rows_split.empty() ? 0 : int64_t(L.rows_split.back()) - L.rows_split.front();
    cols = L.cols_split.empty() ? 0 : int64_t(L.cols_split.back()) - L.cols_split.front();
}

void check_mx_job(const job& j) {
    const costa_dtype_t a = j.A->dtype, c = j.C->dtype;
    if (!mx_pair(a, c))
        throw error(COSTA_ERR_ARG, std::string("costa_hip_transform_mx: no MX transform for ") + dtype_name(a) +
                                       " -> " + dtype_name(c) +
                                       (dtype_is_fp4(a) || dtype_is_fp4(c)
                                            ? " (FLOAT -> FP4_E2M1, FP4_E2M1 -> FLOAT, FP4_E2M1 -> FP4_E2M1)"
                                            : " (FLOAT -> FP8, FP8 -> FLOAT, FP8 -> the same FP8)"));
    if (j.uplo != 'A') throw error(COSTA_ERR_ARG, "costa_hip_transform_mx: no triangular mask");
    if (j.A == j.C) throw error(COSTA_ERR_ARG, "costa_hip_transform_mx: in-place calls are not supported");
    const bool want_a = dtype_is_fp8(a) || dtype_is_fp4(a), want_c = dtype_is_fp8(c) || dtype_is_fp4(c);
    if (want_a && !j.a_scales.data)
        throw error(COSTA_ERR_ARG, std::string("costa_hip_transform_mx: a_scales is required for ") + dtype_name(a) +
                                       " -> " + dtype_name(c));
    if (!want_a && j.a_scales.data)
        throw error(COSTA_ERR_ARG, std::string("costa_hip_transform_mx: a_scales given for a FLOAT source (") +
                                       dtype_name(a) + " -> " + dtype_name(c) + ")");
    if (want_c && !j.c_scales.data)
        throw error(COSTA_ERR_ARG, std::string("costa_hip_transform_mx: c_scales is required for ") + dtype_name(a) +
                                       " -> " + dtype_name(c));
    if (!want_c && j.c_scales.data)
        throw error(COSTA_ERR_ARG, std::string("costa_hip_transform_mx: c_scales given for a FLOAT destination (") +
                                       dtype_name(a) + " -> " + dtype_name(c) + ")");
    if (j.mx_rounding != COSTA_MX_FLOOR && j.mx_rounding != COSTA_MX_CEIL)
        throw error(COSTA_ERR_ARG, "costa_hip_transform_mx: rounding must be COSTA_MX_FLOOR or COSTA_MX_CEIL");
    if (want_c) {
        float beta;
        std::memcpy(&beta, j.s.beta.data(), sizeof beta);
        if (!(beta == 0.0f)) throw error(COSTA_ERR_ARG, "costa_hip_transform_mx: beta must be 0 with c_scales");
    }
    int64_t r, k;
    if (want_a) {
        layout_extent(*j.A, r, k);
        check_mx_scales(j.a_scales, r, k, "costa_hip_transform_mx: a_scales");
    }
    if (want_c) {
        layout_extent(*j.C, r, k);
        check_mx_scales(j.c_scales, r, k, "costa_hip_transform_mx: c_scales");
    }
}

mx_side mx_side_of(const costa_mx_scales_t& s, bool swap) {
    mx_side o;
    o.data = s.data;
    o.block_stride = s.block_stride;
    o.line_stride = s.line_stride;
    o.rows = (s.axis == COSTA_MX_ROWS) != swap;
    return o;
}

void mx_args(const job& j, cached_plan& cp, scaled_args& sv) {
    for (const void* v : {static_cast<const void*>(j.a_scales.data), static_cast<const void*>(j.c_scales.data)})
        if (v && !is_device_ptr(v))
            throw error(COSTA_ERR_ARG, "costa_hip_transform_mx: the scale tensors must be device-resident");
    if (j.c_scales.data) {
        int& ok = cp.mx_rule[j.c_scales.axis == COSTA_MX_ROWS ? 0 : 1];
        int64_t m, n;
        layout_extent(*j.C, m, n);
        if (ok <= 0) {
            ok = -1;
            check_mx_ops(cp.p->local_scaled, j.c_scales.axis, m, n);
            check_mx_ops(cp.p->unpack_scaled, j.c_scales.axis, m, n);
            ok = 1;
        }
    }
    sv = scaled_args{};
    sv.mx = true;
    sv.a_scales = mx_side_of(j.a_scales, std::toupper(static_cast<unsigned char>(j.trans)) != 'N');
    sv.c_scales = mx_side_of(j.c_scales, false);
    sv.ceil = j.mx_rounding == COSTA_MX_CEIL;
}

void launch_local(const cached_plan& cp, const scaled_args& sv, phase_timer& tm, hipStream_t ls) {
    const plan& p = *cp.p;
    if (cp.c_local.n_items) {
        tm.start(PH_LOCAL, ls);
        launch_convert(p.src_dtype, p.dtype, static_cast<const costa_tile_op_t*>(cp.d_local.p),
                       static_cast<const uint64_t*>(cp.w_local.p), cp.c_local, nullptr, nullptr,
                       cp.d_scal.p, ls);
        tm.stop();
    }
    if (cp.l_local.n_items()) {
        tm.start(PH_LOCAL, ls);
        launch_tiles(p.dtype,
                     make_launch(cp.l_local, cp.d_local.p, cp.w_local.p, nullptr, nullptr,
                                 cp.d_scal.p, cp.tr_local, cp.ax_local),
                     ls);
        tm.stop();
    }
    if (cp.t_local.n_items) {
        tm.start(PH_TRI_LOCAL, ls);
        launch_tri(p.dtype, static_cast<const costa_tri_op_t*>(cp.d_local_tri.p),
                   static_cast<const uint64_t*>(cp.w_local_tri.p), cp.t_local, nullptr, nullptr,
                   cp.d_scal.p, ls);
        tm.stop();
    }

    if (cp.s_local.n_items) {
        tm.start(PH_LOCAL, ls);
        if (sv.mx)
            launch_mx(p.src_dtype, p.dtype, static_cast<const costa_scaled_op_t*>(cp.d_local_sc.p),
                      static_cast<const uint64_t*>(cp.w_local_sc.p), cp.s_local, nullptr, nullptr,
                      cp.d_scal.p, sv.a_scales, sv.c_scales, sv.ceil, ls);
        else
            launch_scaled(p.src_dtype, p.dtype, static_cast<const costa_scaled_op_t*>(cp.d_local_sc.p),
                          static_cast<const uint64_t*>(cp.w_local_sc.p), cp.s_local, nullptr, nullptr,
                          cp.d_scal.p, sv.row_scale, sv.col_scale, sv.row_amax, sv.col_amax, ls);
        tm.stop();
    }
}

void launch_pack_round(const cached_plan& cp, const cached_plan::xround& x, char* sb, phase_timer& tm,
                       hipStream_t s) {
    const plan& p = *cp.p;
    if (x.c_pack.n_items) {
        tm.start(PH_PACK, s);
        launch_convert(pack_src(p), pack_dst(p), static_cast<const costa_tile_op_t*>(x.d_pack.p),
                       static_cast<const uint64_t*>(x.w_pack.p), x.c_pack, nullptr, sb,
                       cp.d_scal.p, s);
        tm.stop();
    }
    if (x.l_pack.n_items()) {
        tm.start(PH_PACK, s);
        launch_tiles(p.pkg_dtype,
                     make_launch(x.l_pack, x.d_pack.p, x.w_pack.p, nullptr, sb, cp.d_scal.p,
                                 false, false),
                     s);
        tm.stop();
    }
}

void launch_unpack_round(const cached_plan& cp, const cached_plan::xround& x, const char* rb,
                         const scaled_args& sv, phase_timer& tm, hipStream_t s, hipEvent_t moved) {
    const plan& p = *cp.p;
    if (x.c_unpack.n_items) {
        if (moved) HIP_CHECK(hipStreamWaitEvent(s, moved, 0));
        tm.start(PH_UNPACK, s);
        launch_convert(p.pkg_dtype, p.dtype, static_cast<const costa_tile_op_t*>(x.d_unpack.p),
                       static_cast<const uint64_t*>(x.w_unpack.p), x.c_unpack, rb, nullptr,
                       cp.d_scal.p, s);
        tm.stop();
    }
    if (x.l_unpack.n_items()) {
        if (moved) HIP_CHECK(hipStreamWaitEvent(s, moved, 0));
        tm.start(PH_UNPACK, s);
        launch_tiles(p.dtype,
                     make_launch(x.l_unpack, x.d_unpack.p, x.w_unpack.p, rb, nullptr,
                                 cp.d_scal.p, x.tr_unpack, x.ax_unpack),
                     s);
        tm.stop();
    }
    if (x.t_unpack.n_items) {
        if (moved) HIP_CHECK(hipStreamWaitEvent(s, moved, 0));
        tm.start(PH_TRI_UNPACK, s);
        launch_tri(p.dtype, static_cast<const costa_tri_op_t*>(x.d_unpack_tri.p),
                   static_cast<const uint64_t*>(x.w_unpack_tri.p), x.t_unpack, rb, nullptr,
                   cp.d_scal.p, s);
        tm.stop();
    }
    if (x.s_unpack.n_items) {
        if (moved) HIP_CHECK(hipStreamWaitEvent(s, moved, 0));
        tm.start(PH_UNPACK, s);
        if (sv.mx)
            launch_mx(p.pkg_dtype, p.dtype, static_cast<const costa_scaled_op_t*>(x.d_unpack_sc.p),
                      static_cast<const uint64_t*>(x.w_unpack_sc.p), x.s_unpack, rb, nullptr,
                      cp.d_scal.p, sv.a_scales, sv.c_scales, sv.ceil, s);
        else
            launch_scaled(p.pkg_dtype, p.dtype, static_cast<const costa_scaled_op_t*>(x.d_unpack_sc.p),
                          static_cast<const uint64_t*>(x.w_unpack_sc.p), x.s_unpack, rb, nullptr,
                          cp.d_scal.p, sv.row_scale, sv.col_scale, sv.row_amax, sv.col_amax, s);
        tm.stop();
    }
}

void count_items(const plan& p, const work_split& w) {
    g_stats.tile_items += w.n_large + w.n_medium;
    g_stats.skew_items += w.n_skew;
    g_stats.cblock_items += w.n_cblock;
    g_stats.tiny_items += w.n_tiny;
    if (!dtype_is_complex(p.dtype) && pieces_in_group_launch(w.n_cblock, w.n_tiny))
        g_stats.fused_pieces += w.n_tiny;
}

void count_local(const cached_plan& cp, bool amax, bool mx) {
    const plan& p = *cp.p;
    g_stats.tri_items += cp.t_local.n_items;
    (mx ? g_mx_items : g_scaled_items) += cp.s_local.n_items;
    if (amax) g_amax_items += cp.s_local.n_items;
    if (cp.l_local.n_items() || cp.c_local.n_items || cp.t_local.n_items || cp.s_local.n_items) {
        g_stats.local_launches++;
        g_stats.local_bytes += p.local_bytes;
        count_items(p, cp.l_local);
        g_stats.convert_items += cp.c_local.n_items;
    }
}

void count_pack_round(const cached_plan& cp, const cached_plan::xround& x) {
    g_stats.pack_launches += x.l_pack.n_items() || x.c_pack.n_items ? 1 : 0;
    count_items(*cp.p, x.l_pack);
    g_stats.convert_items += x.c_pack.n_items;
}

void count_unpack_round(const cached_plan& cp, const cached_plan::xround& x, bool amax, bool mx) {
    g_stats.unpack_launches +=
        x.l_unpack.n_items() || x.c_unpack.n_items || x.t_unpack.n_items || x.s_unpack.n_items ? 1 : 0;
    g_stats.tri_items += x.t_unpack.n_items;
    (mx ? g_mx_items : g_scaled_items) += x.s_unpack.n_items;
    if (amax) g_amax_items += x.s_unpack.n_items;
    count_items(*cp.p, x.l_unpack);
    g_stats.convert_items += x.c_unpack.n_items;
}

bool buffer_holds(const void* buffer, size_t bytes) {
    hipDeviceptr_t base = nullptr;
    size_t sz = 0;
    if (hipMemGetAddressRange(&base, &sz, const_cast<void*>(buffer)) != hipSuccess) {
        (void)hipGetLastError();
        return true;
    }
    const size_t off = size_t(static_cast<const char*>(buffer) - static_cast<const char*>(base));
    return off <= sz && sz - off >= bytes;
}

void run_emulated_part(const comm* c, device_ctx& dc, const cached_plan& cp, const scaled_args& sv) {
    const plan& p = *cp.p;
    const size_t E = pkg_unit_size(p.pkg_dtype);
    phase_timer tm(dc, g_profiling);
    const int R = int(cp.rounds.size());
    const int r0 = c->round < 0 ? 0 : c->round, r1 = c->round < 0 ? R : c->round + 1;
    if (c->part == COSTA_EMULATE_LOCAL) {
        launch_local(cp, sv, tm, dc.main);
        count_local(cp, sv.amax(), sv.mx);
        g_stats.transforms++;
    } else if (c->part == COSTA_EMULATE_PACK) {
        if (!buffer_holds(c->buffer, size_t(p.send_elems) * E))
            throw error(COSTA_ERR_ARG, "costa: the emulated send package is smaller than the plan's");
        for (int r = r0; r < r1; ++r) {
            launch_pack_round(cp, *cp.rounds[size_t(r)], static_cast<char*>(c->buffer), tm, dc.main);
            count_pack_round(cp, *cp.rounds[size_t(r)]);
        }
        if (r1 == R) g_stats.pack_bytes += p.pack_bytes;
    } else {
        if (!buffer_holds(c->buffer, size_t(p.recv_elems) * E))
            throw error(COSTA_ERR_ARG, "costa: the emulated receive package is smaller than the plan's");
        for (int r = r0; r < r1; ++r) {
            launch_unpack_round(cp, *cp.rounds[size_t(r)], static_cast<const char*>(c->buffer), sv, tm,
                                dc.main, nullptr);
            count_unpack_round(cp, *cp.rounds[size_t(r)], sv.amax(), sv.mx);
        }
        if (r1 == R) g_stats.unpack_bytes += p.unpack_bytes;
    }
    HIP_CHECK(hipStreamSynchronize(dc.main));
    dc.resolve();
}

}

void transform(const std::vector<job>& jobs, comm* c, void* user_stream, bool async) {
    std::lock_guard<std::recursive_mutex> lk(g_mutex);
    if (!c) throw error(COSTA_ERR_ARG, "costa: null communicator");
    device_ctx& dc = ctx(c->device);
    if (c->emulated) {
        if (c->part == 0)
            throw error(COSTA_ERR_ARG, "costa: an emulated communicator with no part selected "
                                       "(costa_hip_comm_emulate)");
        if (async)
            throw error(COSTA_ERR_ARG, "costa: an emulated communicator runs blocking transforms only "
                                       "(no _async form)");
        for (const job& j : jobs)
            if (!layout_on_device(*j.A) || !layout_on_device(*j.C))
                throw error(COSTA_ERR_ARG, "costa: an emulated communicator needs device-resident layouts");
    }
    const bool mx = jobs.size() == 1 && jobs[0].mx;
    if (!mx && any_fp4(jobs)) {
        costa_dtype_t a, b;
        check_jobs(jobs, c->size, a, b);
    }
    if (mx) check_mx_job(jobs[0]);
    cached_plan& cp = *get_plan(jobs, c, dc);
    const plan& p = *cp.p;
    const size_t E = pkg_unit_size(p.pkg_dtype);
    const void* row_scale = p.scaled ? jobs[0].row_scale : nullptr;
    const void* col_scale = p.scaled ? jobs[0].col_scale : nullptr;
    void* row_amax = p.scaled ? jobs[0].row_amax : nullptr;
    void* col_amax = p.scaled ? jobs[0].col_amax : nullptr;
    const bool amax = row_amax || col_amax;
    scaled_args sv;
    sv.row_scale = row_scale;
    sv.col_scale = col_scale;
    sv.row_amax = row_amax;
    sv.col_amax = col_amax;
    if (mx) {
        mx_args(jobs[0], cp, sv);
    } else if (p.scaled) {
        if (!row_scale && !col_scale && !amax)
            throw error(COSTA_ERR_ARG, "costa: a scaled transform without scale vectors (use costa_hip_transform)");
        for (const void* v : {row_scale, col_scale})
            if (v && !is_device_ptr(v))
                throw error(COSTA_ERR_ARG, "costa: the scale vectors of a scaled transform must be "
                                           "device-resident");
        for (const void* v : {row_amax, col_amax})
            if (v && !is_device_ptr(v))
                throw error(COSTA_ERR_ARG, "costa: the amax vectors of a scaled transform must be "
                                           "device-resident");
    }
    if (async && (cp.staged || cp.pipe))
        throw error(COSTA_ERR_ARG,
                    "costa: asynchronous transforms need device-resident layouts (host data is "
                    "staged synchronously)");
    hipStream_t user = static_cast<hipStream_t>(user_stream);
    if (user) {
        HIP_CHECK(hipEventRecord(dc.ev_user, user));
        HIP_CHECK(hipStreamWaitEvent(dc.main, dc.ev_user, 0));
    }
    upload_scalars(cp, jobs, dc.main);
    if (cp.pipe) {
        const bool xchg = c->nccl != nullptr && (p.send_elems > 0 || p.recv_elems > 0);
        char *sb = nullptr, *rb = nullptr;
        std::function<void(void*, int)> fn;
        if (xchg) {
            dc.send.reserve(size_t(p.send_elems) * E + 256);
            dc.recv.reserve(size_t(p.recv_elems) * E + 256);
            sb = static_cast<char*>(dc.send.p);
            rb = static_cast<char*>(dc.recv.p);
            const int R = exchange_rounds();
            fn = [&, R](void* s, int r) {
                issue_exchange(c, p, sb, rb, static_cast<hipStream_t>(s), r, R);
            };
        }
        HIP_CHECK(hipEventRecord(dc.ev_ready, dc.main));
        HIP_CHECK(hipStreamWaitEvent(dc.aux, dc.ev_ready, 0));
        run_host_pipeline(*cp.pipe, c->device, dc.aux, dc.main, sb, rb, fn, cp.d_scal.p);
        g_stats.transforms++;
        return;
    }
    if (c->emulated) return run_emulated_part(c, dc, cp, sv);
    phase_timer tm(dc, g_profiling);

    if (cp.staged) {
        tm.start(PH_H2D, dc.main);
        for (const auto& r : cp.h2d_ranges)
            HIP_CHECK(hipMemcpyAsync(static_cast<char*>(cp.stage.p) + r.dev_off,
                                     reinterpret_cast<void*>(r.lo), r.hi - r.lo,
                                     hipMemcpyHostToDevice, dc.main));
        tm.stop();
    }

    const bool exchange = c->nccl != nullptr && (p.send_elems > 0 || p.recv_elems > 0);
    hipStream_t ls = exchange ? dc.aux : dc.main;
    if (exchange) {
        HIP_CHECK(hipEventRecord(dc.ev_ready, dc.main));
        HIP_CHECK(hipStreamWaitEvent(dc.aux, dc.ev_ready, 0));
    }
    launch_local(cp, sv, tm, ls);

    if (exchange) {
        dc.send.reserve(size_t(p.send_elems) * E + 256);
        dc.recv.reserve(size_t(p.recv_elems) * E + 256);
        char* sb = static_cast<char*>(dc.send.p);
        char* rb = static_cast<char*>(dc.recv.p);
        const int R = int(cp.rounds.size());
        dc.round_events(size_t(R));
        for (int r = 0; r < R; ++r) {
            launch_pack_round(cp, *cp.rounds[size_t(r)], sb, tm, dc.main);
            HIP_CHECK(hipEventRecord(dc.ev_packed[size_t(r)], dc.main));
            HIP_CHECK(hipStreamWaitEvent(dc.xch, dc.ev_packed[size_t(r)], 0));
            tm.start(PH_EXCHANGE, dc.xch);
            issue_exchange(c, p, sb, rb, dc.xch, r, R);
            tm.stop();
            HIP_CHECK(hipEventRecord(dc.ev_moved[size_t(r)], dc.xch));
        }
        for (int r = 0; r < R; ++r)
            launch_unpack_round(cp, *cp.rounds[size_t(r)], rb, sv, tm, dc.aux, dc.ev_moved[size_t(r)]);
        HIP_CHECK(hipEventRecord(dc.ev_local, dc.aux));
        HIP_CHECK(hipStreamWaitEvent(dc.main, dc.ev_local, 0));
        HIP_CHECK(hipStreamWaitEvent(dc.main, dc.ev_moved[size_t(R - 1)], 0));
    }

    if (cp.staged) {
        tm.start(PH_D2H, dc.main);
        for (const auto& r : cp.d2h_ranges)
            HIP_CHECK(hipMemcpyAsync(reinterpret_cast<void*>(r.lo),
                                     static_cast<char*>(cp.stage.p) + r.dev_off, r.hi - r.lo,
                                     hipMemcpyDeviceToHost, dc.main));
        tm.stop();
    }

    g_stats.transforms++;
    count_local(cp, amax, sv.mx);
    if (exchange) {
        for (const auto& x : cp.rounds) {
            count_pack_round(cp, *x);
            count_unpack_round(cp, *x, amax, sv.mx);
        }
        g_stats.pack_bytes += p.pack_bytes;
        g_stats.unpack_bytes += p.unpack_bytes;
    }

    if (async) {
        if (user) {
            HIP_CHECK(hipEventRecord(dc.ev_done, dc.main));
            HIP_CHECK(hipStreamWaitEvent(user, dc.ev_done, 0));
        }
        return;
    }
    HIP_CHECK(hipStreamSynchronize(dc.main));
    dc.resolve();
}


void execute_tiles(costa_dtype_t dtype, const costa_tile_op_t* ops, int64_t n,
                   const void* src_base, void* dst_base, const void* scalars, int n_slots,
                   int device) {
    std::lock_guard<std::recursive_mutex> lk(g_mutex);
    if (dtype_is_half(dtype) || dtype_is_fp8(dtype) || dtype_is_fp4(dtype))
        throw error(COSTA_ERR_ARG, std::string("costa_hip_execute_tiles: no same-type tile kernel for ") +
                                       dtype_name(dtype) + " (use costa_hip_execute_tiles_mixed)");
    device_ctx& dc = ctx(device);
    std::vector<costa_tile_op_t> v(ops, ops + n);
    for (const auto& op : v)
        if ((op.flags >> COSTA_SLOT_SHIFT) >= uint32_t(std::max(n_slots, 0)))
            throw error(COSTA_ERR_ARG, "costa_hip_execute_tiles: scalar slot out of range");
    std::vector<costa_tile_op_t> ord;
    std::vector<uint64_t> w;
    const work_split nl = build_work(dtype, v, ord, w);
    dbuf d_ops, d_work, d_scal;
    d_ops.upload(ord, dc.main);
    d_work.upload(w, dc.main);
    const size_t E = dtype_size(dtype);
    std::vector<unsigned char> sc(static_cast<const unsigned char*>(scalars),
                                  static_cast<const unsigned char*>(scalars) + size_t(n_slots) * 2 * E);
    d_scal.upload(sc, dc.main);
    launch_tiles(dtype,
                 make_launch(nl, d_ops.p, d_work.p, static_cast<const char*>(src_base),
                             static_cast<char*>(dst_base), d_scal.p, any_transpose(v),
                             any_axpby(v)),
                 dc.main);
    HIP_CHECK(hipStreamSynchronize(dc.main));
}

namespace {
const pair_family& family_of(costa_dtype_t src, costa_dtype_t dst) {
    static const pair_family table[] = {half_family(), fp8_family(), wide_family()};
    for (const pair_family& f : table)
        if (f.has(src, dst)) return f;
    throw error(COSTA_ERR_ARG, std::string("costa: no converting kernel for ") + dtype_name(src) + " -> " +
                                   dtype_name(dst));
}
}

void convert_subtile(costa_dtype_t src, costa_dtype_t dst, int* bf, int* bs) {
    family_of(src, dst).subtile(src, dst, bf, bs);
}

strip_list build_convert_work(costa_dtype_t src_dtype, costa_dtype_t dst_dtype,
                              const std::vector<costa_tile_op_t>& ops, uint64_t src_base, uint64_t dst_base,
                              std::vector<costa_tile_op_t>& ordered, std::vector<uint64_t>& work) {
    int bf = 0, bs = 0;
    convert_subtile(src_dtype, dst_dtype, &bf, &bs);
    const uint64_t es = dtype_size(src_dtype), ed = dtype_size(dst_dtype);
    return build_strip_work("converting", ops, src_base, dst_base, bf, bs, es, ed,
                            strip_alignment(strip_family::pair, es, ed), ordered, work);
}

void launch_convert(costa_dtype_t src_dtype, costa_dtype_t dst_dtype, const costa_tile_op_t* d_ops,
                    const uint64_t* d_work, const strip_list& l, const char* src_base, char* dst_base,
                    const void* d_scalars, void* stream) {
    if (l.n_items <= 0) return;
    family_of(src_dtype, dst_dtype).launch(src_dtype, dst_dtype, d_ops, d_work, l, src_base, dst_base, d_scalars,
                                           stream);
}

namespace {
template <typename Op, typename Build, typename Launch>
int64_t run_strip_tiles(const std::string& who, const Op* ops, int64_t n, const void* scalars, int n_slots,
                        size_t scalar_size, int device, Build build, Launch launch) {
    device_ctx& dc = ctx(device);
    std::vector<Op> v(ops, ops + n);
    for (const Op& t : v)
        if ((tile_of(t).flags >> COSTA_SLOT_SHIFT) >= uint32_t(std::max(n_slots, 0)))
            throw error(COSTA_ERR_ARG, who + ": scalar slot out of range");
    std::vector<Op> ord;
    std::vector<uint64_t> w;
    const strip_list l = build(v, ord, w);
    if (!l.n_items) return 0;
    dbuf d_ops, d_work, d_scal;
    d_ops.upload(ord, dc.main);
    d_work.upload(w, dc.main);
    std::vector<unsigned char> sc(static_cast<const unsigned char*>(scalars),
                                  static_cast<const unsigned char*>(scalars) + size_t(n_slots) * 2 * scalar_size);
    d_scal.upload(sc, dc.main);
    launch(static_cast<const Op*>(d_ops.p), static_cast<const uint64_t*>(d_work.p), l, d_scal.p, dc.main);
    HIP_CHECK(hipStreamSynchronize(dc.main));
    return l.n_items;
}
}

void execute_tiles_mixed(costa_dtype_t src_dtype, costa_dtype_t dst_dtype, const costa_tile_op_t* ops,
                         int64_t n, const void* src_base, void* dst_base, const void* scalars,
                         int n_slots, int device) {
    std::lock_guard<std::recursive_mutex> lk(g_mutex);
    if (!convertible(src_dtype, dst_dtype))
        throw error(COSTA_ERR_ARG, std::string("costa_hip_execute_tiles_mixed: cannot convert ") +
                                       dtype_name(src_dtype) + " to " + dtype_name(dst_dtype) +
                                       " (FLOAT <-> DOUBLE, CFLOAT <-> CDOUBLE, and HALF or BFLOAT16 with "
                                       "itself or FLOAT only, and FP8_E4M3 or FP8_E5M2 with itself or FLOAT)");
    const uintptr_t sb = reinterpret_cast<uintptr_t>(src_base), db = reinterpret_cast<uintptr_t>(dst_base);
    g_stats.convert_items += run_strip_tiles(
        "costa_hip_execute_tiles_mixed", ops, n, scalars, n_slots,
        dtype_size(compute_dtype(src_dtype, dst_dtype)),
        device, [&](const auto& v, auto& ord, auto& w) { return build_convert_work(src_dtype, dst_dtype, v, sb, db, ord, w); },
        [&](const costa_tile_op_t* d_ops, const uint64_t* d_work, const strip_list& l, const void* d_scal, void* s) {
            launch_convert(src_dtype, dst_dtype, d_ops, d_work, l, static_cast<const char*>(src_base),
                           static_cast<char*>(dst_base), d_scal, s);
        });
}

void execute_tiles_tri(costa_dtype_t dtype, const costa_tri_op_t* ops, int64_t n, const void* src_base,
                       void* dst_base, const void* scalars, int n_slots, int device) {
    std::lock_guard<std::recursive_mutex> lk(g_mutex);
    if (dtype_is_half(dtype) || dtype_is_fp8(dtype) || dtype_is_fp4(dtype))
        throw error(COSTA_ERR_ARG, std::string("costa_hip_execute_tiles_tri: no edge-tile kernel for ") +
                                       dtype_name(dtype));
    const uintptr_t sb = reinterpret_cast<uintptr_t>(src_base), db = reinterpret_cast<uintptr_t>(dst_base);
    g_stats.tri_items += run_strip_tiles(
        "costa_hip_execute_tiles_tri", ops, n, scalars, n_slots, dtype_size(dtype), device,
// ... 270 lines not shown
```

costa_amd/csrc/engine.hpp:

```cpp
#pragma once

#include <costa/layout.hpp>
#include <costa_hip.h>

#include <array>
#include <cstdint>
#include <functional>
#include <memory>
#include <string>
#include <vector>

#include "tile_op.hpp"

namespace costa {
namespace engine {

size_t dtype_size(costa_dtype_t t);
esize elem_size(costa_dtype_t t);
bool dtype_is_complex(costa_dtype_t t);
bool dtype_is_half(costa_dtype_t t);
costa_dtype_t compute_dtype(costa_dtype_t src, costa_dtype_t dst);
bool half_pair(costa_dtype_t src, costa_dtype_t dst);
bool dtype_is_fp8(costa_dtype_t t);
bool fp8_pair(costa_dtype_t src, costa_dtype_t dst);
bool dtype_is_fp4(costa_dtype_t t);
bool fp4_pair(costa_dtype_t src, costa_dtype_t dst);
size_t pkg_unit_size(costa_dtype_t pkg);
int64_t pkg_units(costa_dtype_t pkg, int64_t elems);
costa_dtype_t plan_pkg_dtype(costa_dtype_t src, costa_dtype_t dst);

struct eblock {
    interval rows, cols;
    char* data = nullptr;
    int ld = 0;
};

struct elayout {
    costa_dtype_t dtype = COSTA_DOUBLE;
    std::vector<int> rows_split, cols_split;
    std::vector<int> owners;
    int n_ranks = 1;
    char ordering = 'C';
    std::vector<eblock> blocks;
    uint64_t hash = 0;
    uint64_t hash2 = 0;

    int nbr() const { return int(rows_split.size()) - 1; }
    int nbc() const { return int(cols_split.size()) - 1; }
};

template <typename T>
costa_dtype_t dtype_of();

template <typename T>
elayout erase(const grid_layout<T>& L);

uint64_t layout_hash(const elayout& L);
void layout_hashes(const elayout& L, uint64_t& h1, uint64_t& h2);
void set_layout_hash(elayout& L);

struct scal {
    std::array<unsigned char, 16> alpha{};
    std::array<unsigned char, 16> beta{};
};

struct job {
    const elayout* A = nullptr;
    const elayout* C = nullptr;
    char trans = 'N';
    scal s;
    char uplo = 'A';
    int k = 0;
    bool scaled = false;
    const void* row_scale = nullptr;
    const void* col_scale = nullptr;
    void* row_amax = nullptr;
    void* col_amax = nullptr;
    bool mx = false;
    costa_mx_scales_t a_scales{};
    costa_mx_scales_t c_scales{};
    int mx_rounding = 0;
};

struct plan {
    costa_dtype_t dtype = COSTA_DOUBLE;
    costa_dtype_t src_dtype = COSTA_DOUBLE;
    costa_dtype_t pkg_dtype = COSTA_DOUBLE;
    bool mixed() const { return src_dtype != dtype; }
    bool half() const { return dtype_is_half(src_dtype) || dtype_is_half(dtype); }
    bool fp8() const { return dtype_is_fp8(src_dtype) || dtype_is_fp8(dtype); }
    bool fp4() const { return dtype_is_fp4(src_dtype) || dtype_is_fp4(dtype); }
    bool converting() const { return mixed() || half() || fp8() || fp4(); }
    costa_dtype_t scalar_dtype() const { return compute_dtype(src_dtype, dtype); }
    int rank = 0, n_ranks = 1;
    std::vector<costa_tile_op_t> local_ops, pack_ops, unpack_ops;
    std::vector<costa_tri_op_t> local_tri, unpack_tri;
    bool scaled = false;
    std::vector<costa_scaled_op_t> local_scaled, unpack_scaled;
    std::vector<int64_t> send_counts, send_displs, recv_counts, recv_displs;
    int64_t send_elems = 0, recv_elems = 0, local_elems = 0;
    std::vector<scal> slots;
    int64_t local_bytes = 0, pack_bytes = 0, unpack_bytes = 0;
};

struct job_params {
    bool transpose, conj, a_cm, c_cm;
    uint32_t kind_copy, kind_tr;
};
std::vector<job_params> check_jobs(const std::vector<job>& jobs, int n_ranks, costa_dtype_t& dtype);
std::vector<job_params> check_jobs(const std::vector<job>& jobs, int n_ranks,
                                   costa_dtype_t& src_dtype, costa_dtype_t& dst_dtype);
const char* dtype_name(costa_dtype_t t);
bool any_masked(const std::vector<job>& jobs);
constexpr int kTriCut = 256;
bool any_scaled(const std::vector<job>& jobs);
bool scaled_pair(costa_dtype_t src, costa_dtype_t dst);
bool any_mixed(const std::vector<job>& jobs);
bool any_half(const std::vector<job>& jobs);
bool any_fp8(const std::vector<job>& jobs);
bool any_fp4(const std::vector<job>& jobs);

std::unique_ptr<plan> make_plan(const std::vector<job>& jobs, int rank, int n_ranks,
                                int loopback = 0);

std::unique_ptr<plan> make_plan_device(const std::vector<job>& jobs, int rank, int n_ranks,
                                       int loopback, int device, void* stream);
int planner_mode();
void set_planner_mode(int mode);

int loopback_exchange();

const char* tuning_env(const char* name);

size_t max_message_bytes();

int exchange_rounds();
size_t round_min_bytes();
void round_range(int64_t n, size_t E, int R, int r, int64_t& lo, int64_t& hi);

costa_tile_op_t make_tile_op(int n_rows, int n_cols, uint64_t src, int src_stride, bool src_cm,
                             uint64_t dst, int dst_stride, bool dst_cm, bool transpose, bool conj,
                             uint32_t scale_kind, uint32_t slot, size_t elem);
costa_tile_op_t make_tile_op(int n_rows, int n_cols, uint64_t src, int src_stride, bool src_cm,
                             uint64_t dst, int dst_stride, bool dst_cm, bool transpose, bool conj,
                             uint32_t scale_kind, uint32_t slot, size_t src_elem, size_t dst_elem);

uint32_t scale_kind(costa_dtype_t dtype, const scal& s, bool copy_mode, bool conj);

int device_count();
int rccl_version();
struct comm;
struct comm* comm_self(int device);
struct comm* comm_create(const unsigned char* id, int nranks, int rank, int device);
struct comm* comm_emulated(int rank, int nranks, int device);
void comm_emulate(struct comm* c, int part, int round, void* buffer);
void comm_unique_id(unsigned char* out);
int comm_rank(const struct comm* c);
int comm_size(const struct comm* c);
void comm_destroy(struct comm* c);

void transform(const std::vector<job>& jobs, struct comm* c, void* user_stream = nullptr,
               bool async = false);
void synchronize(struct comm* c);
void resolve_pending();
double tri_phase_ms(bool reset);

void copy_and_transform(costa_dtype_t dtype, int n_rows, int n_cols, const void* src,
                        int src_stride, bool src_cm, void* dst, int dst_stride, bool dst_cm,
                        bool trans, bool conj, const void* alpha, const void* beta);

void execute_tiles(costa_dtype_t dtype, const costa_tile_op_t* ops, int64_t n,
                   const void* src_base, void* dst_base, const void* scalars, int n_slots,
                   int device);
void execute_tiles_mixed(costa_dtype_t src_dtype, costa_dtype_t dst_dtype, const costa_tile_op_t* ops,
                         int64_t n, const void* src_base, void* dst_base, const void* scalars,
                         int n_slots, int device);

struct strip_list {
    int64_t n_items = 0;
    bool any_transpose = false;
};

struct pair_family {
    bool (*has)(costa_dtype_t src, costa_dtype_t dst);
    void (*subtile)(costa_dtype_t src, costa_dtype_t dst, int* bf, int* bs);
    void (*launch)(costa_dtype_t src_dtype, costa_dtype_t dst_dtype, const costa_tile_op_t* d_ops,
                   const uint64_t* d_work, const strip_list& l, const char* src_base, char* dst_base,
                   const void* d_scalars, void* stream );
};
bool wide_pair(costa_dtype_t src, costa_dtype_t dst);
pair_family wide_family(), half_family(), fp8_family();
bool convertible(costa_dtype_t src, costa_dtype_t dst);
void convert_subtile(costa_dtype_t src, costa_dtype_t dst, int* bf, int* bs);
strip_list build_convert_work(costa_dtype_t src_dtype, costa_dtype_t dst_dtype,
                              const std::vector<costa_tile_op_t>& ops, uint64_t src_base,
                              uint64_t dst_base, std::vector<costa_tile_op_t>& ordered,
                              std::vector<uint64_t>& work);
void launch_convert(costa_dtype_t src_dtype, costa_dtype_t dst_dtype, const costa_tile_op_t* d_ops,
                    const uint64_t* d_work, const strip_list& l, const char* src_base,
                    char* dst_base, const void* d_scalars, void* stream );

void tri_subtile(costa_dtype_t dtype, int* bf, int* bs);
strip_list build_tri_work(costa_dtype_t dtype, const std::vector<costa_tri_op_t>& ops, uint64_t src_base,
                        uint64_t dst_base, std::vector<costa_tri_op_t>& ordered,
                        std::vector<uint64_t>& work);
void launch_tri(costa_dtype_t dtype, const costa_tri_op_t* d_ops, const uint64_t* d_work,
                const strip_list& l, const char* src_base, char* dst_base, const void* d_scalars,
                void* stream );
void execute_tiles_tri(costa_dtype_t dtype, const costa_tri_op_t* ops, int64_t n, const void* src_base,
                       void* dst_base, const void* scalars, int n_slots, int device);

void scaled_subtile(costa_dtype_t src, costa_dtype_t dst, int* bf, int* bs);
strip_list build_scaled_work(costa_dtype_t src_dtype, costa_dtype_t dst_dtype,
                             const std::vector<costa_scaled_op_t>& ops, uint64_t src_base,
                             uint64_t dst_base, std::vector<costa_scaled_op_t>& ordered,
                             std::vector<uint64_t>& work, bool dst_order);
void launch_scaled(costa_dtype_t src_dtype, costa_dtype_t dst_dtype, const costa_scaled_op_t* d_ops,
                   const uint64_t* d_work, const strip_list& l, const char* src_base, char* dst_base,
                   const void* d_scalars, const void* row_scale, const void* col_scale, void* row_amax,
                   void* col_amax, void* stream );
void execute_tiles_scaled(costa_dtype_t src_dtype, costa_dtype_t dst_dtype, const costa_scaled_op_t* ops,
                          int64_t n, const void* src_base, void* dst_base, const void* scalars,
                          int n_slots, const void* row_scale, const void* col_scale, int device);
int64_t scaled_items(bool reset);
void execute_tiles_amax(costa_dtype_t src_dtype, costa_dtype_t dst_dtype, const costa_scaled_op_t* ops,
                        int64_t n, const void* src_base, void* dst_base, const void* scalars,
                        int n_slots, const void* row_scale, const void* col_scale, void* row_amax,
                        void* col_amax, int device);
bool amax_dtype(costa_dtype_t t);
std::vector<costa_scaled_op_t> layout_amax_ops(const elayout& L);
void launch_amax(costa_dtype_t dtype, const costa_scaled_op_t* d_ops, const uint64_t* d_work,
                 int64_t n_items, void* row_amax, void* col_amax, void* stream );
void layout_amax(const elayout& L, void* row_amax, void* col_amax, struct comm* c, void* user_stream,
                 bool async);
int64_t amax_items(bool reset);
struct mx_side {
    void* data = nullptr;
    int64_t block_stride = 0, line_stride = 0;
    bool rows = true;
};
bool mx_pair(costa_dtype_t src, costa_dtype_t dst);
void check_fp4_ops(costa_dtype_t src_dtype, costa_dtype_t dst_dtype, const std::vector<costa_scaled_op_t>& ops);
void launch_mx(costa_dtype_t src_dtype, costa_dtype_t dst_dtype, const costa_scaled_op_t* d_ops,
               const uint64_t* d_work, const strip_list& l, const char* src_base, char* dst_base,
               const void* d_scalars, const mx_side& a_scales, const mx_side& c_scales, bool ceil,
               void* stream );
void check_mx_scales(const costa_mx_scales_t& s, int64_t rows, int64_t cols, const std::string& what);
void check_mx_ops(const std::vector<costa_scaled_op_t>& ops, int axis, int64_t m, int64_t n);
void execute_tiles_mx(costa_dtype_t src_dtype, costa_dtype_t dst_dtype, const costa_scaled_op_t* ops,
                      int64_t n_ops, const void* src_base, void* dst_base, const void* scalars, int n_slots,
                      const costa_mx_scales_t* a_scales, const costa_mx_scales_t* c_scales, int rounding,
                      int64_t m, int64_t n, int a_transposed, int device);
int64_t mx_items(bool reset);
void exchange_round_of_scaled(const struct plan& p, int rounds, std::vector<int>& unpack_round);

constexpr int kTinyCopyBytes = 16384;
constexpr int kTinyLdsBytes = 8192;
constexpr int kTinyLdsDefault = 4096;
int64_t tiny_lds_budget();
constexpr int tiny_copy_lane_bytes(size_t) { return 64; }
int64_t tiny_copy_budget(int64_t elem_size, bool local_list = true);
constexpr int64_t kUnalignedWaveCap = 4;
constexpr int tiny_lds_bytes = kTinyLdsBytes;

struct launch_args {
    const costa_tile_op_t* ops;
    const uint64_t* work;
    int64_t n_large;
    int64_t n_medium;
    int64_t n_skew = 0;
    int64_t n_cblock = 0;
    int64_t cblock_lds = 0;
    int cb_map = 0;
    int64_t tiny_first;
    int64_t n_tiny;
    const char* src_base;
    char* dst_base;
    const void* scalars;
    bool any_transpose;
    bool any_axpby;
    bool tr_shape;
    bool sq;
    bool full;
    bool med_full;
    bool med_sq;
    bool skew_wide = false;
};
bool any_transpose(const std::vector<costa_tile_op_t>& ops);
bool any_axpby(const std::vector<costa_tile_op_t>& ops);
void launch_tiles(costa_dtype_t dtype, const launch_args& a, void* stream );
bool pieces_in_group_launch(int64_t n_cblock, int64_t n_tiny);
constexpr int64_t kPanelBytes = int64_t(128) << 10;
constexpr int kCblockThreads = 256;
constexpr int kCblockChunks = 4;
inline int64_t cblock_max_elems(int64_t E) { return int64_t(kCblockThreads) * kCblockChunks * (16 / E); }
constexpr int64_t kCblockXcdChunk = 16;
constexpr int64_t cblock_xcd_order(int64_t b, int64_t nb, int64_t ch = kCblockXcdChunk) {
    return b / (8 * ch) * (8 * ch) + 8 * ch <= nb ? b / (8 * ch) * (8 * ch) + (b % 8) * ch + (b / 8) % ch : b;
}
constexpr int64_t xcd_slice_order(int64_t b, int64_t nb) {
    return (b % 8) < nb % 8 ? (b % 8) * (nb / 8 + 1) + b / 8
                            : (nb % 8) * (nb / 8 + 1) + ((b % 8) - nb % 8) * (nb / 8) + b / 8;
}
enum cblock_map { cb_round_robin = 0, cb_xcd_chunks = 1, cb_xcd_bands = 2 };
struct shape_dims {
    int bf = 0, bs = 0, bf_m = 0, bs_m = 0, bf_q = 0, bs_q = 0, bf_s = 0, bs_s = 0;
    int cf = 0, cs = 0;
    int bf_k = 0, bs_k = 0;
    int bf_kw = 0, bs_kw = 0;
};
void tile_shapes(costa_dtype_t dtype, bool transposing_list, shape_dims* out);
struct work_split {
    int64_t n_large = 0, n_medium = 0, tiny_first = 0, n_tiny = 0;
    int64_t n_skew = 0;
    int64_t n_cblock = 0;
    int64_t cblock_lds = 0;
    int cb_map = 0;
    bool tr_shape = false;
    bool sq = false;
    bool full = false;
    bool med_full = false;
    bool med_sq = false;
    bool skew_wide = false;
    int64_t n_items() const { return n_large + n_medium + n_skew + n_cblock + n_tiny; }
};
enum list_kind { list_local, list_pack, list_unpack };
struct device_section {
    int device = -1;
    void* stream = nullptr;
    bool force = false;
    std::shared_ptr<void> mem;
    costa_tile_op_t* d_ordered = nullptr;
    uint64_t* d_work = nullptr;
    size_t at_ordered = 0, n_ordered = 0, at_work = 0, n_work = 0;
};
work_split build_work(costa_dtype_t dtype, const std::vector<costa_tile_op_t>& ops,
                      std::vector<costa_tile_op_t>& ordered, std::vector<uint64_t>& work,
                      list_kind kind = list_local, device_section* dev = nullptr, bool dst_order = false);
constexpr size_t kDeviceGroupsMin = 16384;
int list_builder_mode();
void set_list_builder_mode(int mode);
int64_t cblock_groups_device(int64_t E, int64_t budget, uint32_t vec_bits, int bands_env,
                             const std::vector<costa_tile_op_t>& ops, const std::vector<uint32_t>& wave,
                             size_t base_at, device_section& sec, std::vector<char>& taken,
                             int64_t& lds, int& map);
bool work_export(costa_dtype_t dtype, const std::vector<costa_tile_op_t>& ops, list_kind kind,
                 int device, std::vector<costa_tile_op_t>& ordered, std::vector<uint64_t>& work,
                 work_split& w);
launch_args make_launch(const work_split& w, const void* d_ordered, const void* d_work,
                        const char* src_base, char* dst_base, const void* d_scalars, bool transpose,
                        bool axpby);

struct host_pipeline;
bool host_pipeline_accepts(costa_dtype_t dtype, const std::vector<costa_tile_op_t>& pack_ops);
std::shared_ptr<host_pipeline> make_host_pipeline(costa_dtype_t dtype,
                                                  const std::vector<costa_tile_op_t>& pack_ops,
                                                  const std::vector<costa_tile_op_t>& local_ops,
                                                  const std::vector<costa_tile_op_t>& unpack_ops,
                                                  const std::vector<int>& pack_round,
                                                  const std::vector<int>& unpack_round, int rounds);
size_t host_pipeline_groups(const host_pipeline& hp);
void run_host_pipeline(host_pipeline& hp, int device, void* compute_stream, void* exchange_stream,
                       char* send_buf, char* recv_buf,
                       const std::function<void(void*, int)>& exchange, const void* d_scalars);
void exchange_round_of_ops(const struct plan& p, int rounds, std::vector<int>& pack_round,
                           std::vector<int>& unpack_round);
void exchange_round_of_tri(const struct plan& p, int rounds, std::vector<int>& unpack_tri_round);
void release_host_rings();
int host_staging_mode();
void set_host_staging_mode(int mode);

struct error : std::runtime_error {
    int code;
    error(int c, const std::string& m) : std::runtime_error(m), code(c) {}
};

costa_stats_t& stats();
bool profiling();
void set_profiling(bool on);
void release_caches();

}
}
```

include/costa_hip.h:

```cpp
#ifndef COSTA_HIP_H
#define COSTA_HIP_H

#include <stddef.h>
#include <stdint.h>

#ifdef __cplusplus
extern "C" {
#endif

#define COSTA_OK 0
#define COSTA_ERR_ARG 1
#define COSTA_ERR_HIP 2
#define COSTA_ERR_NCCL 3
#define COSTA_ERR_INTERNAL 4

typedef enum {
    COSTA_FLOAT = 0,
    COSTA_DOUBLE = 1,
    COSTA_CFLOAT = 2,
    COSTA_CDOUBLE = 3,
    COSTA_INT32 = 4,
    COSTA_HALF = 5,
    COSTA_BFLOAT16 = 6,
    COSTA_FP8_E4M3 = 7,
// ... 108 lines not shown
                             void* row_amax, void* col_amax, costa_comm_t comm);
int costa_hip_transform_amax_async(costa_layout_t A, costa_layout_t C, char trans, const void* alpha,
                                   const void* beta, const void* row_scale, const void* col_scale,
                                   void* row_amax, void* col_amax, costa_comm_t comm, void* stream);
int costa_hip_layout_amax(costa_layout_t A, void* row_amax, void* col_amax, costa_comm_t comm);
int costa_hip_layout_amax_async(costa_layout_t A, void* row_amax, void* col_amax, costa_comm_t comm,
                                void* stream);

#define COSTA_MX_ROWS 0
#define COSTA_MX_COLS 1
#define COSTA_MX_FLOOR 0
#define COSTA_MX_CEIL 1
typedef struct {
    void* data;
    int axis;
    int64_t block_stride;
    int64_t line_stride;
} costa_mx_scales_t;
int costa_hip_transform_mx(costa_layout_t A, costa_layout_t C, char trans, const void* alpha,
                           const void* beta, const costa_mx_scales_t* a_scales,
                           const costa_mx_scales_t* c_scales, int rounding, costa_comm_t comm);
int costa_hip_transform_mx_async(costa_layout_t A, costa_layout_t C, char trans, const void* alpha,
                                 const void* beta, const costa_mx_scales_t* a_scales,
                                 const costa_mx_scales_t* c_scales, int rounding, costa_comm_t comm,
                                 void* stream);
int costa_hip_execute_tiles_mx(costa_dtype_t src_dtype, costa_dtype_t dst_dtype,
                               const costa_scaled_op_t* ops, int64_t n_ops, const void* src_base,
                               void* dst_base, const void* scalars, int n_slots,
                               const costa_mx_scales_t* a_scales, const costa_mx_scales_t* c_scales,
                               int rounding, int64_t m, int64_t n, int a_transposed, int device);
int costa_hip_mx_items(int64_t* items, int reset);
int costa_hip_mx_check_ops(const costa_scaled_op_t* ops, int64_t n_ops, int axis, int64_t m, int64_t n);
int costa_hip_mx_check_scales(const costa_mx_scales_t* s, int64_t rows, int64_t cols);


int costa_hip_transform_async(costa_layout_t A, costa_layout_t C, char trans, const void* alpha,
                              const void* beta, costa_comm_t comm, void* stream);
int costa_hip_transform_batch_async(int n, const costa_layout_t* A, const costa_layout_t* C,
                                    const char* trans, const void* alpha, const void* beta,
                                    costa_comm_t comm, void* stream);
int costa_hip_synchronize(costa_comm_t comm);

int costa_hip_copy_and_transform(costa_dtype_t dtype, int n_rows, int n_cols, const void* src,
                                 int src_stride, int src_col_major, void* dst, int dst_stride,
                                 int dst_col_major, int transpose, int conjugate,
                                 const void* alpha, const void* beta);
int costa_hip_execute_tiles(costa_dtype_t dtype, const costa_tile_op_t* ops, int64_t n,
                            const void* src_base, void* dst_base, const void* scalars,
                            int n_slots, int device);
int costa_hip_execute_tiles_mixed(costa_dtype_t src_dtype, costa_dtype_t dst_dtype,
                                  const costa_tile_op_t* ops, int64_t n, const void* src_base,
                                  void* dst_base, const void* scalars, int n_slots, int device);
int costa_hip_convert_subtile(costa_dtype_t src_dtype, costa_dtype_t dst_dtype, int* bf, int* bs);

int costa_hip_execute_tiles_tri(costa_dtype_t dtype, const costa_tri_op_t* ops, int64_t n,
                                const void* src_base, void* dst_base, const void* scalars,
                                int n_slots, int device);
int costa_hip_tri_cut(void);
int costa_hip_tri_subtile(costa_dtype_t dtype, int* bf, int* bs);

int costa_hip_execute_tiles_scaled(costa_dtype_t src_dtype, costa_dtype_t dst_dtype,
                                   const costa_scaled_op_t* ops, int64_t n, const void* src_base,
                                   void* dst_base, const void* scalars, int n_slots,
                                   const void* row_scale, const void* col_scale, int device);
int costa_hip_scaled_subtile(costa_dtype_t src_dtype, costa_dtype_t dst_dtype, int* bf, int* bs);
int costa_hip_scaled_items(int64_t* items, int reset);
int costa_hip_execute_tiles_amax(costa_dtype_t src_dtype, costa_dtype_t dst_dtype,
                                 const costa_scaled_op_t* ops, int64_t n, const void* src_base,
                                 void* dst_base, const void* scalars, int n_slots,
                                 const void* row_scale, const void* col_scale, void* row_amax,
                                 void* col_amax, int device);
int costa_hip_amax_items(int64_t* items, int reset);

typedef struct {
    int64_t n_local;
    int64_t n_pack;
    int64_t n_unpack;
    int64_t send_elems;
    int64_t recv_elems;
    int64_t local_elems;
    int32_t n_ranks;
    int32_t n_slots;
} costa_plan_info_t;

int costa_hip_plan_export(int n, const costa_layout_t* A, const costa_layout_t* C,
                          const char* trans, const void* alpha, const void* beta, int rank,
                          int nranks, costa_plan_info_t* info, costa_tile_op_t* local_ops,
                          costa_tile_op_t* pack_ops, costa_tile_op_t* unpack_ops,
                          int64_t* send_counts, int64_t* send_displs, int64_t* recv_counts,
                          int64_t* recv_displs, void* scalars);

typedef struct {
    costa_plan_info_t base;
    int64_t n_local_tri;
    int64_t n_unpack_tri;
} costa_tri_plan_info_t;
int costa_hip_plan_export_tri(costa_layout_t A, costa_layout_t C, char trans, char uplo, int k,
                              const void* alpha, const void* beta, int rank, int nranks,
                              costa_tri_plan_info_t* info, costa_tile_op_t* local_ops,
                              costa_tile_op_t* pack_ops, costa_tile_op_t* unpack_ops,
                              costa_tri_op_t* local_tri, costa_tri_op_t* unpack_tri,
                              int64_t* send_counts, int64_t* send_displs, int64_t* recv_counts,
                              int64_t* recv_displs, void* scalars);

typedef struct {
    costa_plan_info_t base;
    int64_t n_local_scaled;
    int64_t n_unpack_scaled;
} costa_scaled_plan_info_t;
int costa_hip_plan_export_scaled(costa_layout_t A, costa_layout_t C, char trans, const void* alpha,
                                 const void* beta, int rank, int nranks,
                                 costa_scaled_plan_info_t* info, costa_tile_op_t* pack_ops,
                                 costa_scaled_op_t* local_scaled, costa_scaled_op_t* unpack_scaled,
                                 int64_t* send_counts, int64_t* send_displs, int64_t* recv_counts,
                                 int64_t* recv_displs, void* scalars);

typedef struct {
    double pack_ms, local_ms, unpack_ms, exchange_ms, h2d_ms, d2h_ms;
    int64_t pack_launches, local_launches, unpack_launches;
    int64_t pack_bytes, local_bytes, unpack_bytes;
    int64_t transforms;
    int64_t plan_hits, plan_misses;
    int64_t host_groups;
    int64_t device_plans;
    double plan_ms;
    int64_t host_direct;
    int64_t host_direct_groups;
    int64_t tile_items, skew_items, cblock_items, tiny_items;
    int64_t device_lists;
    int64_t fused_pieces;
    int64_t convert_items;
    int64_t tri_items;
} costa_stats_t;
int costa_hip_tri_phase_ms(double* ms, int reset);
int costa_hip_set_profiling(int on);
int costa_hip_get_stats(costa_stats_t* out, int reset);
int costa_hip_release_caches(void);

int costa_hip_set_host_staging(int mode);

int costa_hip_set_planner(int mode);
int costa_hip_plan_export_device(int device, int n, const costa_layout_t* A, const costa_layout_t* C,
                                 const char* trans, const void* alpha, const void* beta, int rank,
                                 int nranks, costa_plan_info_t* info, costa_tile_op_t* local_ops,
                                 costa_tile_op_t* pack_ops, costa_tile_op_t* unpack_ops,
                                 int64_t* send_counts, int64_t* send_displs, int64_t* recv_counts,
                                 int64_t* recv_displs, void* scalars);

int costa_hip_set_list_builder(int mode);
int costa_hip_work_export(int dtype, const costa_tile_op_t* ops, int64_t n_ops, int kind, int device,
                          costa_tile_op_t* ordered, int64_t cap_ordered, uint64_t* work,
                          int64_t cap_work, int64_t* meta);

#ifdef __cplusplus
}
#endif
#endif
```

Measured before the change: 6209 GB/s.

## Share cached transform plans across buffers with identical geometry via base-relative rebasing

Plans now store tile operations as offsets relative to an aligned base of the source and destination layouts, with the bases passed to the kernels at launch. A new layout geometry hash ignores absolute addresses, so a call on different device buffers with the same shape can reuse an existing plan body instead of replanning. This targets plan-building cost when buffers change between calls. It adds pointer-attribute queries on a cache miss and extra base arithmetic in the kernels; a steady-state benchmark that reuses the same buffers would see little change.

```diff
diff --git a/costa_amd/__init__.py b/costa_amd/__init__.py
--- a/costa_amd/__init__.py
+++ b/costa_amd/__init__.py
@@ -261,6 +261,9 @@
                                              vp]),
         "costa_hip_set_list_builder": (i, [i]),
         "costa_hip_work_export": (i, [i, vp, i64, i, i, vp, i64, vp, i64, C.POINTER(i64)]),
+        "costa_hip_shared_plans": (i, [C.POINTER(i64), i]),
+        "costa_hip_layout_geometry_key": (i, [vp, C.POINTER(C.c_uint64), C.POINTER(C.c_uint64)]),
+        "costa_hip_work_rebase": (i, [vp, i64, vp, i64, C.POINTER(i64), C.c_uint64, C.c_uint64]),
     }
     for name, (res, args) in sig.items():
         try:
@@ -1001,6 +1004,29 @@
     return WorkLists(o, w, m, bool(m["on_gpu"]))
 
 
+def shared_plans(reset: bool = False) -> int:
+    n = C.c_int64(0)
+    _check(lib().costa_hip_shared_plans(C.byref(n), int(reset)))
+    return n.value
+
+
+def layout_geometry_key(layout: "Layout") -> tuple:
+    k = (C.c_uint64 * 2)()
+    b = C.c_uint64(0)
+    _check(lib().costa_hip_layout_geometry_key(layout.handle, k, C.byref(b)))
+    return int(k[0]), int(k[1]), int(b.value)
+
+
+def work_rebase(w: WorkLists, src_shift: int, dst_shift: int) -> np.ndarray:
+    o = np.ascontiguousarray(w.ordered, dtype=TILE_OP_DTYPE).copy()
+    k = np.ascontiguousarray(w.work, dtype=np.uint64)
+    meta = (C.c_int64 * 12)(*[int(w.meta[n]) for n in _WORK_META])
+    m64 = (1 << 64) - 1
+    _check(lib().costa_hip_work_rebase(o.ctypes.data, o.size, k.ctypes.data, k.size, meta,
+                                       int(src_shift) & m64, int(dst_shift) & m64))
+    return o
+
+
 def set_host_staging(mode: int):
     _check(lib().costa_hip_set_host_staging(int(mode)))
 
diff --git a/costa_amd/csrc/capi.cpp b/costa_amd/csrc/capi.cpp
--- a/costa_amd/csrc/capi.cpp
+++ b/costa_amd/csrc/capi.cpp
@@ -871,6 +871,42 @@
     return device >= 0 ? gpu_guarded(body) : guarded(body);
 }
 
+int costa_hip_shared_plans(int64_t* count, int reset) {
+    return guarded([&] {
+        if (!count) throw costa::engine::error(COSTA_ERR_ARG, "null argument");
+        *count = costa::engine::shared_plans(reset != 0);
+    });
+}
+
+int costa_hip_layout_geometry_key(costa_layout_t layout, uint64_t key[2], uint64_t* base) {
+    return guarded([&] {
+        if (!layout || !key) throw costa::engine::error(COSTA_ERR_ARG, "null argument");
+        key[0] = layout->e.ghash;
+        key[1] = layout->e.ghash2;
+        if (base) *base = layout->e.base;
+    });
+}
+
+int costa_hip_work_rebase(costa_tile_op_t* ordered, int64_t n_ordered, const uint64_t* work,
+                          int64_t n_work, const int64_t* meta, uint64_t src_shift, uint64_t dst_shift) {
+    return guarded([&] {
+        if (!meta || n_ordered < 0 || n_work < 0 || (n_ordered > 0 && !ordered) || (n_work > 0 && !work))
+            throw costa::engine::error(COSTA_ERR_ARG, "null argument");
+        costa::engine::work_split ws;
+        ws.n_large = meta[0];
+        ws.n_medium = meta[1];
+        ws.n_skew = meta[2];
+        ws.n_cblock = meta[3];
+        if (ws.n_large < 0 || ws.n_medium < 0 || ws.n_skew < 0 || ws.n_cblock < 0 ||
+            ws.n_large + ws.n_medium + ws.n_skew + ws.n_cblock > n_work)
+            throw costa::engine::error(COSTA_ERR_ARG, "costa: the counts in meta exceed the work list");
+        std::vector<costa_tile_op_t> o(ordered, ordered + n_ordered);
+        const std::vector<uint64_t> w(work, work + n_work);
+        costa::engine::rebase_work(o, w, ws, src_shift, dst_shift);
+        if (n_ordered > 0) std::memcpy(ordered, o.data(), o.size() * sizeof(o[0]));
+    });
+}
+
 int costa_hip_set_profiling(int on) {
     costa::engine::set_profiling(on != 0);
     return COSTA_OK;
diff --git a/costa_amd/csrc/device_lists.hip b/costa_amd/csrc/device_lists.hip
--- a/costa_amd/csrc/device_lists.hip
+++ b/costa_amd/csrc/device_lists.hip
@@ -706,5 +706,34 @@
     return ng;
 }
 
-}
-}
+namespace {
+__global__ void dl_rebase(costa_tile_op_t* ops, int64_t n, uint64_t src_shift, uint64_t dst_shift) {
+    const int64_t i = int64_t(blockIdx.x) * blockDim.x + threadIdx.x;
+    if (i >= n) return;
+    ops[i].src -= src_shift;
+    ops[i].dst -= dst_shift;
+}
+__global__ void dl_rebase_headers(costa_tile_op_t* ops, int64_t n, const uint64_t* work, int64_t ng, uint64_t first,
+                                  uint64_t src_shift) {
+    const int64_t q = int64_t(blockIdx.x) * blockDim.x + threadIdx.x;
+    if (q >= ng) return;
+    const uint64_t h = work[q] - first;
+    if (h < uint64_t(n)) ops[h].src += src_shift;
+}
+}
+
+void rebase_device_section(const device_section& sec, uint64_t src_shift, uint64_t dst_shift) {
+    if (!sec.n_ordered || !sec.d_ordered) return;
+    hipStream_t s = static_cast<hipStream_t>(sec.stream);
+    const int64_t n = int64_t(sec.n_ordered), ng = int64_t(sec.n_work);
+    hipLaunchKernelGGL(dl_rebase, dim3(dl_grid(n)), dim3(kThreads), 0, s, sec.d_ordered, n, src_shift, dst_shift);
+    DL_CHECK(hipGetLastError());
+    if (ng > 0 && src_shift) {
+        hipLaunchKernelGGL(dl_rebase_headers, dim3(dl_grid(ng)), dim3(kThreads), 0, s, sec.d_ordered, n, sec.d_work, ng,
+                           uint64_t(sec.at_ordered), src_shift);
+        DL_CHECK(hipGetLastError());
+    }
+}
+
+}
+}
diff --git a/costa_amd/csrc/engine.cpp b/costa_amd/csrc/engine.cpp
--- a/costa_amd/csrc/engine.cpp
+++ b/costa_amd/csrc/engine.cpp
@@ -1415,6 +1415,17 @@
     return a;
 }
 
+void rebase_work(std::vector<costa_tile_op_t>& ordered, const std::vector<uint64_t>& work, const work_split& w,
+                 uint64_t src_shift, uint64_t dst_shift) {
+    for (auto& op : ordered) {
+        op.src -= src_shift;
+        op.dst -= dst_shift;
+    }
+    const size_t g0 = size_t(w.n_large + w.n_medium + w.n_skew);
+    for (size_t q = g0; q < std::min(work.size(), g0 + size_t(w.n_cblock)); ++q)
+        if (work[q] < ordered.size()) ordered[size_t(work[q])].src += src_shift;
+}
+
 namespace {
 
 struct hrange {
@@ -1498,7 +1509,7 @@
         mix(v.size());
         for (int x : v) mix(uint64_t(uint32_t(x)));
     }
-    void mix_layout(const elayout& L) {
+    void mix_layout(const elayout& L, uint64_t origin) {
         mix(uint64_t(L.dtype));
         mix(uint64_t(uint8_t(L.ordering)));
         mix(uint64_t(L.n_ranks));
@@ -1509,34 +1520,65 @@
         for (const auto& b : L.blocks) {
             mix(uint64_t(uint32_t(b.rows.start)) | (uint64_t(uint32_t(b.rows.end)) << 32));
             mix(uint64_t(uint32_t(b.cols.start)) | (uint64_t(uint32_t(b.cols.end)) << 32));
-            mix(reinterpret_cast<uintptr_t>(b.data));
+            mix(reinterpret_cast<uintptr_t>(b.data) - origin);
             mix(uint64_t(uint32_t(b.ld)));
         }
     }
 };
 
-}
-
-uint64_t layout_hash(const elayout& L) {
+constexpr uint64_t kRebaseAlign = 256;
+
+}
+
+namespace {
+void hash_layout(const elayout& L, uint64_t& h1, uint64_t& h2, uint64_t& g1, uint64_t& g2, uint64_t& base,
+                 uint64_t& ext_hi) {
+    base = L.blocks.empty() ? 0 : ~uint64_t(0);
+    ext_hi = 0;
+    const esize E = elem_size(L.dtype);
+    for (const auto& b : L.blocks) {
+        const uint64_t lo = reinterpret_cast<uintptr_t>(b.data);
+        const int64_t nr = b.rows.length(), nc = b.cols.length();
+        const int64_t fast = L.ordering == 'R' ? nc : nr, slow = L.ordering == 'R' ? nr : nc;
+        const int64_t elems = nr > 0 && nc > 0 ? (slow - 1) * int64_t(b.ld) + fast : 0;
+        base = std::min(base, lo);
+        ext_hi = std::max(ext_hi, lo + (uint64_t(std::max<int64_t>(elems, 0)) * E.hb + 1) / 2);
+    }
     hasher h;
-    h.mix_layout(L);
-    return h.h | 1;
-}
-
-void layout_hashes(const elayout& L, uint64_t& h1, uint64_t& h2) {
-    hasher h;
-    h.mix_layout(L);
+    h.mix_layout(L, base & ~(kRebaseAlign - 1));
+    h.mix(base % kRebaseAlign);
+    g1 = h.h | 1;
+    g2 = h.h2;
+    h.mix(base);
     h1 = h.h | 1;
     h2 = h.h2;
 }
-
-void set_layout_hash(elayout& L) { layout_hashes(L, L.hash, L.hash2); }
+}
+
+uint64_t layout_hash(const elayout& L) {
+    uint64_t h1, h2;
+    layout_hashes(L, h1, h2);
+    return h1;
+}
+
+void layout_hashes(const elayout& L, uint64_t& h1, uint64_t& h2) {
+    uint64_t g1, g2, base, hi;
+    hash_layout(L, h1, h2, g1, g2, base, hi);
+}
+
+void layout_geometry(const elayout& L, uint64_t& g1, uint64_t& g2, uint64_t& base, uint64_t& ext_hi) {
+    uint64_t h1, h2;
+    hash_layout(L, h1, h2, g1, g2, base, ext_hi);
+}
+
+void set_layout_hash(elayout& L) { hash_layout(L, L.hash, L.hash2, L.ghash, L.ghash2, L.base, L.ext_hi); }
 
 namespace {
 
-struct cached_plan {
+struct plan_body {
     std::unique_ptr<plan> p;
     int device = 0;
+    bool rebased = false;
     bool staged = false;
     std::vector<hrange> h2d_ranges, d2h_ranges;
     dbuf stage;
@@ -1565,12 +1607,17 @@
 };
 
 constexpr size_t kMaxPlans = 16;
-struct keyed_plan {
+struct cached_plan {
     uint64_t h = 0;
     std::vector<uint64_t> key;
-    std::unique_ptr<cached_plan> plan;
+    std::shared_ptr<plan_body> body;
+    const char* a_base = nullptr;
+    char* c_base = nullptr;
+    std::vector<uint64_t> gkey;
+    uint64_t a_lo = 0, a_hi = 0, c_lo = 0, c_hi = 0;
 };
-std::list<keyed_plan> g_plans;
+std::list<cached_plan> g_plans;
+int64_t g_shared_plans = 0;
 
 void key_layout(std::vector<uint64_t>& k, const elayout& L) {
     uint64_t h1 = L.hash, h2 = L.hash2;
@@ -1586,6 +1633,60 @@
             k.push_back(reinterpret_cast<uintptr_t>(b->data));
             k.push_back(uint64_t(uint32_t(b->ld)) | uint64_t(uint32_t(b->rows.start)) << 32);
         }
+}
+
+struct layout_geo {
+    uint64_t g1, g2, base, hi;
+};
+layout_geo geo_of(const elayout& L) {
+    layout_geo g{L.ghash, L.ghash2, L.base, L.ext_hi};
+    if (!g.g1) layout_geometry(L, g.g1, g.g2, g.base, g.hi);
+    return g;
+}
+
+void key_geometry(std::vector<uint64_t>& k, const elayout& L, const layout_geo& g) {
+    k.push_back(g.g1);
+    k.push_back(g.g2);
+    k.push_back(uint64_t(L.dtype) | uint64_t(uint8_t(L.ordering)) << 8 |
+                uint64_t(uint32_t(L.n_ranks)) << 32);
+    k.push_back(uint64_t(uint32_t(L.nbr())) | uint64_t(uint32_t(L.nbc())) << 32);
+    k.push_back(L.blocks.size());
+    k.push_back(g.base % kRebaseAlign);
+    if (!L.blocks.empty())
+        for (const eblock* b : {&L.blocks.front(), &L.blocks.back()}) {
+            k.push_back(reinterpret_cast<uintptr_t>(b->data) - (g.base & ~(kRebaseAlign - 1)));
+            k.push_back(uint64_t(uint32_t(b->ld)) | uint64_t(uint32_t(b->rows.start)) << 32);
+        }
+}
+
+bool range_on_device(uint64_t lo, uint64_t hi, int device) {
+    hipPointerAttribute_t a;
+    if (hipPointerGetAttributes(&a, reinterpret_cast<const void*>(lo)) != hipSuccess) {
+        (void)hipGetLastError();
+        return false;
+    }
+    if (a.type != hipMemoryTypeDevice || a.device != device) return false;
+    hipDeviceptr_t base = nullptr;
+    size_t sz = 0;
+    if (hipMemGetAddressRange(&base, &sz, reinterpret_cast<void*>(lo)) != hipSuccess) {
+        (void)hipGetLastError();
+        return false;
+    }
+    return hi <= reinterpret_cast<uintptr_t>(base) + sz;
+}
+
+bool same_overlap(uint64_t a1_lo, uint64_t a1_hi, uint64_t c1_lo, uint64_t c1_hi, uint64_t a2_lo,
+                  uint64_t a2_hi, uint64_t c2_lo, uint64_t c2_hi) {
+    const bool o1 = a1_lo < c1_hi && c1_lo < a1_hi, o2 = a2_lo < c2_hi && c2_lo < a2_hi;
+    return o1 == o2 && (!o1 || c1_lo - a1_lo == c2_lo - a2_lo);
+}
+
+template <typename Op>
+void rebase_ops(std::vector<Op>& ops, uint64_t src_shift, uint64_t dst_shift) {
+    for (auto& o : ops) {
+        tile_of(o).src -= src_shift;
+        tile_of(o).dst -= dst_shift;
+    }
 }
 
 elayout remap(const elayout& L, const std::vector<hrange>& ranges, char* dev) {
@@ -1742,10 +1843,39 @@
         if (it->h == h.h && it->key == key) {
             g_plans.splice(g_plans.begin(), g_plans, it);
             g_stats.plan_hits++;
-            return g_plans.front().plan.get();
+            return &g_plans.front();
         }
     }
     g_stats.plan_misses++;
+    const bool may_share = jobs.size() == 1 && !c->emulated;
+    std::vector<uint64_t> gkey;
+    layout_geo ga{}, gc{};
+    if (may_share) {
+        ga = geo_of(*jobs[0].A);
+        gc = geo_of(*jobs[0].C);
+        gkey.reserve(key.size() + 2);
+        gkey.insert(gkey.end(), key.begin(), key.begin() + 3);
+        key_geometry(gkey, *jobs[0].A, ga);
+        key_geometry(gkey, *jobs[0].C, gc);
+        gkey.insert(gkey.end(), key.end() - 2, key.end());
+        for (auto it = g_plans.begin(); it != g_plans.end(); ++it) {
+            if (it->gkey != gkey || !it->body->rebased) continue;
+            if (!same_overlap(it->a_lo, it->a_hi, it->c_lo, it->c_hi, ga.base, ga.hi, gc.base, gc.hi)) continue;
+            if (!range_on_device(ga.base, ga.hi, c->device) || !range_on_device(gc.base, gc.hi, c->device)) break;
+            cached_plan e;
+            e.h = h.h;
+            e.key = std::move(key);
+            e.body = it->body;
+            e.a_base = reinterpret_cast<const char*>(ga.base & ~(kRebaseAlign - 1));
+            e.c_base = reinterpret_cast<char*>(gc.base & ~(kRebaseAlign - 1));
+            e.gkey = std::move(gkey);
+            e.a_lo = ga.base, e.a_hi = ga.hi, e.c_lo = gc.base, e.c_hi = gc.hi;
+            g_plans.push_front(std::move(e));
+            while (g_plans.size() > kMaxPlans) g_plans.pop_back();
+            g_shared_plans++;
+            return &g_plans.front();
+        }
+    }
     static const bool trace = std::getenv("COSTA_PLAN_TRACE") != nullptr;
     auto now = [] {
         return std::chrono::duration<double, std::milli>(
@@ -1764,8 +1894,16 @@
         costa_dtype_t a, b;
         check_jobs(jobs, c->size, a, b);
     }
-    auto cp = std::make_unique<cached_plan>();
+    auto cp = std::make_shared<plan_body>();
     cp->device = c->device;
+    auto cache = [&](cached_plan&& e) {
+        e.h = h.h;
+        e.key = std::move(key);
+        e.body = std::move(cp);
+        g_plans.push_front(std::move(e));
+        while (g_plans.size() > kMaxPlans) g_plans.pop_back();
+        return &g_plans.front();
+    };
     bool all_dev = true;
     std::vector<const elayout*> host_layouts;
     std::vector<bool> on_dev;
@@ -1850,9 +1988,7 @@
                 exchange_round_of_ops(*cp->p, R, pr, ur);
                 cp->pipe = make_host_pipeline(cp->p->dtype, cp->p->pack_ops, cp->p->local_ops,
                                               cp->p->unpack_ops, pr, ur, R);
-                g_plans.push_front({h.h, std::move(key), std::move(cp)});
-                while (g_plans.size() > kMaxPlans) g_plans.pop_back();
-                return g_plans.front().plan.get();
+                return cache(cached_plan{});
             }
         }
         cp->stage.reserve(std::max<size_t>(off, 256));
@@ -1965,7 +2101,7 @@
     std::vector<std::vector<uint64_t>> w_p(static_cast<size_t>(R)), w_u(static_cast<size_t>(R));
     std::vector<device_section> sec_u(static_cast<size_t>(R), section());
     for (int r = 0; r < R; ++r) {
-        auto x = std::make_unique<cached_plan::xround>();
+        auto x = std::make_unique<plan_body::xround>();
         x->tr_unpack = any_transpose(up[size_t(r)]);
         x->ax_unpack = any_axpby(up[size_t(r)]);
         if (cv_pack)
@@ -1986,6 +2122,27 @@
                                             w_us[size_t(r)], false);
         cp->rounds.push_back(std::move(x));
     }
+    cached_plan entry;
+    if (may_share && all_dev) {
+        const uint64_t sa = ga.base & ~(kRebaseAlign - 1), sd = gc.base & ~(kRebaseAlign - 1);
+        rebase_work(ord_l, w_l, cp->l_local, sa, sd);
+        if (sec_l.n_ordered) rebase_device_section(sec_l, sa, sd);
+        rebase_ops(ord_lt, sa, sd);
+        rebase_ops(ord_ls, sa, sd);
+        for (int r = 0; r < R; ++r) {
+            auto& x = *cp->rounds[size_t(r)];
+            rebase_work(ord_p[size_t(r)], w_p[size_t(r)], x.l_pack, sa, 0);
+            rebase_work(ord_u[size_t(r)], w_u[size_t(r)], x.l_unpack, 0, sd);
+            if (sec_u[size_t(r)].n_ordered) rebase_device_section(sec_u[size_t(r)], 0, sd);
+            rebase_ops(ord_ut[size_t(r)], 0, sd);
+            rebase_ops(ord_us[size_t(r)], 0, sd);
+        }
+        cp->rebased = true;
+        entry.a_base = reinterpret_cast<const char*>(sa);
+        entry.c_base = reinterpret_cast<char*>(sd);
+        entry.gkey = std::move(gkey);
+        entry.a_lo = ga.base, entry.a_hi = ga.hi, entry.c_lo = gc.base, entry.c_hi = gc.hi;
+    }
     t_work = now() - t0 - t_resid - t_plan;
     upload_list(cp->d_local, ord_l, sec_l.d_ordered, sec_l.at_ordered, sec_l.n_ordered, dc.main);
     upload_list(cp->w_local, w_l, sec_l.d_work, sec_l.at_work, sec_l.n_work, dc.main);
@@ -2021,12 +2178,10 @@
                      p.local_ops.size(), p.pack_ops.size(), p.unpack_ops.size(), t_resid, t_plan,
                      t_work, now() - t0 - t_resid - t_plan - t_work, now() - t0);
 
-    g_plans.push_front({h.h, std::move(key), std::move(cp)});
-    while (g_plans.size() > kMaxPlans) g_plans.pop_back();
-    return g_plans.front().plan.get();
-}
-
-void upload_scalars(cached_plan& cp, const std::vector<job>& jobs, hipStream_t s) {
+    return cache(std::move(entry));
+}
+
+void upload_scalars(plan_body& cp, const std::vector<job>& jobs, hipStream_t s) {
     const size_t E = dtype_size(cp.p->scalar_dtype());
     std::vector<unsigned char> host(jobs.size() * 2 * E);
     for (size_t t = 0; t < jobs.size(); ++t) {
@@ -2041,6 +2196,13 @@
     }
 }
 
+}
+
+int64_t shared_plans(bool reset) {
+    std::lock_guard<std::recursive_mutex> lk(g_mutex);
+    const int64_t n = g_shared_plans;
+    if (reset) g_shared_plans = 0;
+    return n;
 }
 
 void release_caches() {
@@ -2226,7 +2388,7 @@
     return o;
 }
 
-void mx_args(const job& j, cached_plan& cp, scaled_args& sv) {
+void mx_args(const job& j, plan_body& cp, scaled_args& sv) {
     for (const void* v : {static_cast<const void*>(j.a_scales.data), static_cast<const void*>(j.c_scales.data)})
         if (v && !is_device_ptr(v))
             throw error(COSTA_ERR_ARG, "costa_hip_transform_mx: the scale tensors must be device-resident");
@@ -2248,19 +2410,20 @@
     sv.ceil = j.mx_rounding == COSTA_MX_CEIL;
 }
 
-void launch_local(const cached_plan& cp, const scaled_args& sv, phase_timer& tm, hipStream_t ls) {
+void launch_local(const cached_plan& e, const scaled_args& sv, phase_timer& tm, hipStream_t ls) {
+    const plan_body& cp = *e.body;
     const plan& p = *cp.p;
     if (cp.c_local.n_items) {
         tm.start(PH_LOCAL, ls);
         launch_convert(p.src_dtype, p.dtype, static_cast<const costa_tile_op_t*>(cp.d_local.p),
-                       static_cast<const uint64_t*>(cp.w_local.p), cp.c_local, nullptr, nullptr,
+                       static_cast<const uint64_t*>(cp.w_local.p), cp.c_local, e.a_base, e.c_base,
                        cp.d_scal.p, ls);
         tm.stop();
     }
     if (cp.l_local.n_items()) {
         tm.start(PH_LOCAL, ls);
         launch_tiles(p.dtype,
-                     make_launch(cp.l_local, cp.d_local.p, cp.w_local.p, nullptr, nullptr,
+                     make_launch(cp.l_local, cp.d_local.p, cp.w_local.p, e.a_base, e.c_base,
                                  cp.d_scal.p, cp.tr_local, cp.ax_local),
                      ls);
         tm.stop();
@@ -2268,7 +2431,7 @@
     if (cp.t_local.n_items) {
         tm.start(PH_TRI_LOCAL, ls);
         launch_tri(p.dtype, static_cast<const costa_tri_op_t*>(cp.d_local_tri.p),
-                   static_cast<const uint64_t*>(cp.w_local_tri.p), cp.t_local, nullptr, nullptr,
+                   static_cast<const uint64_t*>(cp.w_local_tri.p), cp.t_local, e.a_base, e.c_base,
                    cp.d_scal.p, ls);
         tm.stop();
     }
@@ -2277,44 +2440,46 @@
         tm.start(PH_LOCAL, ls);
         if (sv.mx)
             launch_mx(p.src_dtype, p.dtype, static_cast<const costa_scaled_op_t*>(cp.d_local_sc.p),
-                      static_cast<const uint64_t*>(cp.w_local_sc.p), cp.s_local, nullptr, nullptr,
+                      static_cast<const uint64_t*>(cp.w_local_sc.p), cp.s_local, e.a_base, e.c_base,
                       cp.d_scal.p, sv.a_scales, sv.c_scales, sv.ceil, ls);
         else
             launch_scaled(p.src_dtype, p.dtype, static_cast<const costa_scaled_op_t*>(cp.d_local_sc.p),
-                          static_cast<const uint64_t*>(cp.w_local_sc.p), cp.s_local, nullptr, nullptr,
+                          static_cast<const uint64_t*>(cp.w_local_sc.p), cp.s_local, e.a_base, e.c_base,
                           cp.d_scal.p, sv.row_scale, sv.col_scale, sv.row_amax, sv.col_amax, ls);
         tm.stop();
     }
 }
 
-void launch_pack_round(const cached_plan& cp, const cached_plan::xround& x, char* sb, phase_timer& tm,
+void launch_pack_round(const cached_plan& e, const plan_body::xround& x, char* sb, phase_timer& tm,
                        hipStream_t s) {
+    const plan_body& cp = *e.body;
     const plan& p = *cp.p;
     if (x.c_pack.n_items) {
         tm.start(PH_PACK, s);
         launch_convert(pack_src(p), pack_dst(p), static_cast<const costa_tile_op_t*>(x.d_pack.p),
-                       static_cast<const uint64_t*>(x.w_pack.p), x.c_pack, nullptr, sb,
+                       static_cast<const uint64_t*>(x.w_pack.p), x.c_pack, e.a_base, sb,
                        cp.d_scal.p, s);
         tm.stop();
     }
     if (x.l_pack.n_items()) {
         tm.start(PH_PACK, s);
         launch_tiles(p.pkg_dtype,
-                     make_launch(x.l_pack, x.d_pack.p, x.w_pack.p, nullptr, sb, cp.d_scal.p,
+                     make_launch(x.l_pack, x.d_pack.p, x.w_pack.p, e.a_base, sb, cp.d_scal.p,
                                  false, false),
                      s);
         tm.stop();
     }
 }
 
-void launch_unpack_round(const cached_plan& cp, const cached_plan::xround& x, const char* rb,
+void launch_unpack_round(const cached_plan& e, const plan_body::xround& x, const char* rb,
                          const scaled_args& sv, phase_timer& tm, hipStream_t s, hipEvent_t moved) {
+    const plan_body& cp = *e.body;
     const plan& p = *cp.p;
     if (x.c_unpack.n_items) {
         if (moved) HIP_CHECK(hipStreamWaitEvent(s, moved, 0));
         tm.start(PH_UNPACK, s);
         launch_convert(p.pkg_dtype, p.dtype, static_cast<const costa_tile_op_t*>(x.d_unpack.p),
-                       static_cast<const uint64_t*>(x.w_unpack.p), x.c_unpack, rb, nullptr,
+                       static_cast<const uint64_t*>(x.w_unpack.p), x.c_unpack, rb, e.c_base,
                        cp.d_scal.p, s);
         tm.stop();
     }
@@ -2322,7 +2487,7 @@
         if (moved) HIP_CHECK(hipStreamWaitEvent(s, moved, 0));
         tm.start(PH_UNPACK, s);
         launch_tiles(p.dtype,
-                     make_launch(x.l_unpack, x.d_unpack.p, x.w_unpack.p, rb, nullptr,
+                     make_launch(x.l_unpack, x.d_unpack.p, x.w_unpack.p, rb, e.c_base,
                                  cp.d_scal.p, x.tr_unpack, x.ax_unpack),
                      s);
         tm.stop();
@@ -2331,7 +2496,7 @@
         if (moved) HIP_CHECK(hipStreamWaitEvent(s, moved, 0));
         tm.start(PH_TRI_UNPACK, s);
         launch_tri(p.dtype, static_cast<const costa_tri_op_t*>(x.d_unpack_tri.p),
-                   static_cast<const uint64_t*>(x.w_unpack_tri.p), x.t_unpack, rb, nullptr,
+                   static_cast<const uint64_t*>(x.w_unpack_tri.p), x.t_unpack, rb, e.c_base,
                    cp.d_scal.p, s);
         tm.stop();
     }
@@ -2340,11 +2505,11 @@
         tm.start(PH_UNPACK, s);
         if (sv.mx)
             launch_mx(p.pkg_dtype, p.dtype, static_cast<const costa_scaled_op_t*>(x.d_unpack_sc.p),
-                      static_cast<const uint64_t*>(x.w_unpack_sc.p), x.s_unpack, rb, nullptr,
+                      static_cast<const uint64_t*>(x.w_unpack_sc.p), x.s_unpack, rb, e.c_base,
                       cp.d_scal.p, sv.a_scales, sv.c_scales, sv.ceil, s);
         else
             launch_scaled(p.pkg_dtype, p.dtype, static_cast<const costa_scaled_op_t*>(x.d_unpack_sc.p),
-                          static_cast<const uint64_t*>(x.w_unpack_sc.p), x.s_unpack, rb, nullptr,
+                          static_cast<const uint64_t*>(x.w_unpack_sc.p), x.s_unpack, rb, e.c_base,
                           cp.d_scal.p, sv.row_scale, sv.col_scale, sv.row_amax, sv.col_amax, s);
         tm.stop();
     }
@@ -2359,7 +2524,7 @@
         g_stats.fused_pieces += w.n_tiny;
 }
 
-void count_local(const cached_plan& cp, bool amax, bool mx) {
+void count_local(const plan_body& cp, bool amax, bool mx) {
     const plan& p = *cp.p;
     g_stats.tri_items += cp.t_local.n_items;
     (mx ? g_mx_items : g_scaled_items) += cp.s_local.n_items;
@@ -2372,13 +2537,13 @@
     }
 }
 
-void count_pack_round(const cached_plan& cp, const cached_plan::xround& x) {
+void count_pack_round(const plan_body& cp, const plan_body::xround& x) {
     g_stats.pack_launches += x.l_pack.n_items() || x.c_pack.n_items ? 1 : 0;
     count_items(*cp.p, x.l_pack);
     g_stats.convert_items += x.c_pack.n_items;
 }
 
-void count_unpack_round(const cached_plan& cp, const cached_plan::xround& x, bool amax, bool mx) {
+void count_unpack_round(const plan_body& cp, const plan_body::xround& x, bool amax, bool mx) {
     g_stats.unpack_launches +=
         x.l_unpack.n_items() || x.c_unpack.n_items || x.t_unpack.n_items || x.s_unpack.n_items ? 1 : 0;
     g_stats.tri_items += x.t_unpack.n_items;
@@ -2399,21 +2564,22 @@
     return off <= sz && sz - off >= bytes;
 }
 
-void run_emulated_part(const comm* c, device_ctx& dc, const cached_plan& cp, const scaled_args& sv) {
+void run_emulated_part(const comm* c, device_ctx& dc, const cached_plan& e, const scaled_args& sv) {
+    const plan_body& cp = *e.body;
     const plan& p = *cp.p;
     const size_t E = pkg_unit_size(p.pkg_dtype);
     phase_timer tm(dc, g_profiling);
     const int R = int(cp.rounds.size());
     const int r0 = c->round < 0 ? 0 : c->round, r1 = c->round < 0 ? R : c->round + 1;
     if (c->part == COSTA_EMULATE_LOCAL) {
-        launch_local(cp, sv, tm, dc.main);
+        launch_local(e, sv, tm, dc.main);
         count_local(cp, sv.amax(), sv.mx);
         g_stats.transforms++;
     } else if (c->part == COSTA_EMULATE_PACK) {
         if (!buffer_holds(c->buffer, size_t(p.send_elems) * E))
             throw error(COSTA_ERR_ARG, "costa: the emulated send package is smaller than the plan's");
         for (int r = r0; r < r1; ++r) {
-            launch_pack_round(cp, *cp.rounds[size_t(r)], static_cast<char*>(c->buffer), tm, dc.main);
+            launch_pack_round(e, *cp.rounds[size_t(r)], static_cast<char*>(c->buffer), tm, dc.main);
             count_pack_round(cp, *cp.rounds[size_t(r)]);
         }
         if (r1 == R) g_stats.pack_bytes += p.pack_bytes;
@@ -2421,7 +2587,7 @@
         if (!buffer_holds(c->buffer, size_t(p.recv_elems) * E))
             throw error(COSTA_ERR_ARG, "costa: the emulated receive package is smaller than the plan's");
         for (int r = r0; r < r1; ++r) {
-            launch_unpack_round(cp, *cp.rounds[size_t(r)], static_cast<const char*>(c->buffer), sv, tm,
+            launch_unpack_round(e, *cp.rounds[size_t(r)], static_cast<const char*>(c->buffer), sv, tm,
                                 dc.main, nullptr);
             count_unpack_round(cp, *cp.rounds[size_t(r)], sv.amax(), sv.mx);
         }
@@ -2454,7 +2620,8 @@
         check_jobs(jobs, c->size, a, b);
     }
     if (mx) check_mx_job(jobs[0]);
-    cached_plan& cp = *get_plan(jobs, c, dc);
+    const cached_plan& e = *get_plan(jobs, c, dc);
+    plan_body& cp = *e.body;
     const plan& p = *cp.p;
     const size_t E = pkg_unit_size(p.pkg_dtype);
     const void* row_scale = p.scaled ? jobs[0].row_scale : nullptr;
@@ -2511,7 +2678,7 @@
         g_stats.transforms++;
         return;
     }
-    if (c->emulated) return run_emulated_part(c, dc, cp, sv);
+    if (c->emulated) return run_emulated_part(c, dc, e, sv);
     phase_timer tm(dc, g_profiling);
 
     if (cp.staged) {
@@ -2529,7 +2696,7 @@
         HIP_CHECK(hipEventRecord(dc.ev_ready, dc.main));
         HIP_CHECK(hipStreamWaitEvent(dc.aux, dc.ev_ready, 0));
     }
-    launch_local(cp, sv, tm, ls);
+    launch_local(e, sv, tm, ls);
 
     if (exchange) {
         dc.send.reserve(size_t(p.send_elems) * E + 256);
@@ -2539,7 +2706,7 @@
         const int R = int(cp.rounds.size());
         dc.round_events(size_t(R));
         for (int r = 0; r < R; ++r) {
-            launch_pack_round(cp, *cp.rounds[size_t(r)], sb, tm, dc.main);
+            launch_pack_round(e, *cp.rounds[size_t(r)], sb, tm, dc.main);
             HIP_CHECK(hipEventRecord(dc.ev_packed[size_t(r)], dc.main));
             HIP_CHECK(hipStreamWaitEvent(dc.xch, dc.ev_packed[size_t(r)], 0));
             tm.start(PH_EXCHANGE, dc.xch);
@@ -2548,7 +2715,7 @@
             HIP_CHECK(hipEventRecord(dc.ev_moved[size_t(r)], dc.xch));
         }
         for (int r = 0; r < R; ++r)
-            launch_unpack_round(cp, *cp.rounds[size_t(r)], rb, sv, tm, dc.aux, dc.ev_moved[size_t(r)]);
+            launch_unpack_round(e, *cp.rounds[size_t(r)], rb, sv, tm, dc.aux, dc.ev_moved[size_t(r)]);
         HIP_CHECK(hipEventRecord(dc.ev_local, dc.aux));
         HIP_CHECK(hipStreamWaitEvent(dc.main, dc.ev_local, 0));
         HIP_CHECK(hipStreamWaitEvent(dc.main, dc.ev_moved[size_t(R - 1)], 0));
diff --git a/costa_amd/csrc/engine.hpp b/costa_amd/csrc/engine.hpp
--- a/costa_amd/csrc/engine.hpp
+++ b/costa_amd/csrc/engine.hpp
@@ -44,6 +44,8 @@
     std::vector<eblock> blocks;
     uint64_t hash = 0;
     uint64_t hash2 = 0;
+    uint64_t ghash = 0, ghash2 = 0;
+    uint64_t base = 0, ext_hi = 0;
 
     int nbr() const { return int(rows_split.size()) - 1; }
     int nbc() const { return int(cols_split.size()) - 1; }
@@ -58,6 +60,7 @@
 uint64_t layout_hash(const elayout& L);
 void layout_hashes(const elayout& L, uint64_t& h1, uint64_t& h2);
 void set_layout_hash(elayout& L);
+void layout_geometry(const elayout& L, uint64_t& g1, uint64_t& g2, uint64_t& base, uint64_t& ext_hi);
 
 struct scal {
     std::array<unsigned char, 16> alpha{};
@@ -347,6 +350,10 @@
 bool work_export(costa_dtype_t dtype, const std::vector<costa_tile_op_t>& ops, list_kind kind,
                  int device, std::vector<costa_tile_op_t>& ordered, std::vector<uint64_t>& work,
                  work_split& w);
+void rebase_work(std::vector<costa_tile_op_t>& ordered, const std::vector<uint64_t>& work, const work_split& w,
+                 uint64_t src_shift, uint64_t dst_shift);
+void rebase_device_section(const device_section& sec, uint64_t src_shift, uint64_t dst_shift);
+int64_t shared_plans(bool reset);
 launch_args make_launch(const work_split& w, const void* d_ordered, const void* d_work,
                         const char* src_base, char* dst_base, const void* d_scalars, bool transpose,
                         bool axpby);
diff --git a/include/costa_hip.h b/include/costa_hip.h
--- a/include/costa_hip.h
+++ b/include/costa_hip.h
@@ -284,6 +284,11 @@
                           costa_tile_op_t* ordered, int64_t cap_ordered, uint64_t* work,
                           int64_t cap_work, int64_t* meta);
 
+int costa_hip_shared_plans(int64_t* count, int reset);
+int costa_hip_layout_geometry_key(costa_layout_t layout, uint64_t key[2], uint64_t* base);
+int costa_hip_work_rebase(costa_tile_op_t* ordered, int64_t n_ordered, const uint64_t* work,
+                          int64_t n_work, const int64_t* meta, uint64_t src_shift, uint64_t dst_shift);
+
 #ifdef __cplusplus
 }
 #endif
```

Result: no change. 6202 GB/s (-0.1%).
